# jiahuei/sparse-image-captioning

Measured on AMD Instinct MI355X. Metric: captions/sec, higher is better.
Workload: dtype bf16; 1 GPU; configs[1]: ORT dense, 256 images x 5 captions, teacher-forcing XE fwd+bwd+clip+Adam; images_per_gpu=256, regions=36, captions_per_image=5, parallelism=single

## Files before the change

### include/ortk.h

```cpp
#ifndef ORTK_H
#define ORTK_H

#include <stddef.h>
#include <stdint.h>

#ifdef __cplusplus
extern "C" {
#endif

#define ORTK_VERSION 13
#define ORTK_EINVAL (-1)
#define ORTK_ENOSPC (-2)
#define ORTK_ENOSYS (-3)
#define ORTK_EEXCHANGE (-4)

typedef void* ortk_stream;

int ortk_version(void);
int ortk_device_ok(void);

struct ortk_sparse_plan;
typedef struct ortk_config {
    int32_t d_model, d_ff, n_layers, n_heads;
    int32_t vocab, feat, seq_len;
    int32_t pad_id, bos_id, eos_id, unk_id;
    int32_t box_trig;
    int32_t precision;
    float   drop_src, drop;
    int32_t share_enc[16], share_dec[16];
    int32_t share_att_enc, share_att_dec;
    int32_t no_box;
    const struct ortk_sparse_plan* sparse_fwd;
    const struct ortk_sparse_plan* sparse_bwd;
} ortk_config;

int64_t ortk_arena_numel(const ortk_config* cfg);
int64_t ortk_arena_numel_with_buffers(const ortk_config* cfg);
int32_t ortk_arena_entries(const ortk_config* cfg);
int ortk_arena_entry(const ortk_config* cfg, int32_t index, char* name_buf, int64_t* offset,
                     int64_t* numel, int32_t* ndim, int64_t* shape, int32_t* kind);

uint32_t ortk_dropout_site_seed(uint64_t seed, int32_t stack, int32_t layer, int32_t k);

typedef struct ortk_batch {
    const float*   att_feats;
    const float*   boxes;
    const float*   att_masks;
    const int64_t* seqs;
    int64_t        seq_stride;
    const float*   tok_weight;
    int32_t B, S, R, T;
    const int32_t* cap_off;
    const int32_t* row_pos;
    int32_t        Mc;
    int32_t        no_pad_keys;
} ortk_batch;

int ortk_valid_position_tables(const int64_t* counts, int32_t R, int32_t T, int32_t* cap_off, int32_t* row_pos, ortk_stream stream);
size_t ortk_train_workspace_bytes(const ortk_config* cfg, int32_t B, int32_t S, int32_t R, int32_t T);
int ortk_valid_positions_ok(const ortk_config* cfg, int32_t B, int32_t S, int32_t R, int32_t T);

int ortk_forward(const ortk_config* cfg, const float* params, const ortk_batch* batch, void* ws, size_t ws_bytes,
                 float* logp_out, int64_t ldv, int32_t train, uint64_t seed, ortk_stream stream);
int ortk_forward_phase(const ortk_config* cfg, const float* params, const ortk_batch* batch, void* ws, size_t ws_bytes,
                       float* logp_out, int64_t ldv, int32_t train, uint64_t seed, int32_t phase, ortk_stream stream);
void* ortk_train_workspace_memory(const ortk_config* cfg, int32_t B, int32_t S, int32_t R, int32_t T, void* ws, int32_t* dtype);

int ortk_loss(const ortk_config* cfg, const ortk_batch* batch, void* ws, size_t ws_bytes,
              const float* norm_dev, float* loss_dev, ortk_stream stream);

int ortk_loss_smooth(const ortk_config* cfg, const ortk_batch* batch, void* ws, size_t ws_bytes,
                     const float* norm_dev, float* loss_dev, float smoothing, ortk_stream stream);

int ortk_loss_external(const ortk_config* cfg, const ortk_batch* batch, void* ws, size_t ws_bytes,
                       const float* logp, const float* dlogp, int64_t ldv, ortk_stream stream);

int ortk_backward(const ortk_config* cfg, const float* params, float* grads, const ortk_batch* batch,
                  void* ws, size_t ws_bytes, int32_t train, uint64_t seed, ortk_stream stream);
int ortk_backward_phase(const ortk_config* cfg, const float* params, float* grads, const ortk_batch* batch,
                        void* ws, size_t ws_bytes, int32_t train, uint64_t seed, int32_t phase, ortk_stream stream);
int64_t ortk_arena_decoder_offset(const ortk_config* cfg);

#define ORTK_SP_ELL32 0
#define ORTK_SP_ELL16 1
#define ORTK_SP_GU16  2
typedef struct ortk_sparse_block {
    int64_t src_offset;
    int64_t ld;
    int64_t stream_offset;
    int64_t capacity;
    int32_t N, K;
    int32_t chunk0;
    int32_t row0;
} ortk_sparse_block;

typedef struct ortk_sparse_plan {
    const ortk_sparse_block* blocks_host; const ortk_sparse_block* blocks_dev;
    int32_t nblocks, format;
    void* stream;
    int32_t* chunk_ptr;
    int32_t* chunk_len;
    int32_t* perm;
    int32_t* count_scratch;
    int32_t* overflow;
    int64_t total_rows;
} ortk_sparse_plan;

int ortk_sparse_build(const ortk_sparse_plan* plan, const void* dense, int32_t dtype, ortk_stream stream);

typedef struct ortk_spmm_args {
    const void* X; void* Y;
    int64_t ldx, ldy; int64_t M;
    int32_t x_dtype, y_dtype;
    const float* bias; const float* rowscale; const float* resid; int64_t ldr;
    const void* gate; int64_t ldg; int32_t gate_dtype; float gate_scale;
    int32_t relu; float drop_p; uint32_t drop_seed;
    const int32_t* drop_rows;
} ortk_spmm_args;
int ortk_spmm(const ortk_sparse_plan* plan, int32_t block, const ortk_spmm_args* a, ortk_stream stream);
int ortk_spmm_plan(const ortk_sparse_plan* plan, int32_t block, const ortk_spmm_args* a, char* buf, int32_t buf_bytes);

typedef struct ortk_chain_unit { int64_t offset, ld; } ortk_chain_unit;
typedef struct ortk_chain_args {
    const void* w16; const ortk_chain_unit* units_dev; int32_t n_units;
    void* packed; size_t packed_bytes;
    int64_t M;
    const float* x_in;
    const void* a_in; const float* bias_r; float* x_mid; uint32_t seed_r;
    const float *g1, *b1; void* y1; float* st1;
    int32_t n1; const float* bias_s1; void* out1; int64_t ld1;
    int32_t NC; const float *bias_h, *bias_o; void* h; float* x_out; uint32_t seed_h, seed_o;
    const float *g2, *b2; void* y2; float* st2;
    int32_t n2; const float* bias_s2; void* out2; int64_t ld2;
    float drop_p, eps;
    int32_t* progress;
    const int32_t* drop_rows;
} ortk_chain_args;
size_t ortk_chain_packed_bytes(int32_t n_units);
int ortk_row_chain(const ortk_chain_args* a, ortk_stream stream);

typedef struct ortk_bchain_args {
    const void* w16t; const ortk_chain_unit* units_dev; int32_t n_units;
    void* packed; size_t packed_bytes;
    int64_t M;
    int32_t nin; const void* ain; int64_t ld_ain; const void* dz0;
    const float *xa, *sta, *ga, *dresa; float *dxa, *daa, *dba; void* dza; uint32_t seed_a; int32_t mask_a;
    int32_t NC; const void* hgate; void* gh; float gate_scale;
    const float *xb, *stb, *gb, *dresb; float *dxb, *dab, *dbb; void* dzb; uint32_t seed_b; int32_t mask_b;
    int32_t n2; void* out2;
    float drop_p, eps;
    const int32_t* drop_rows;
} ortk_bchain_args;
int ortk_row_bchain(const ortk_bchain_args* a, ortk_stream stream);

typedef struct ortk_tuning {
    int32_t gemm_t64;
    int32_t attn_impl;
    int32_t attn16_min_lq;
    int32_t side_stream;
    int32_t row_chain;
    int32_t chain_wide;
    int32_t spmm_alias;
    int32_t f32_split;
    int32_t wgrad_wgs;
    int32_t wgrad_group;
    int32_t wgrad_group_splitk;
    int32_t wgrad_group_wgs;
    int32_t wgrad_group_tail;
    int32_t feats_bf16;
    int32_t ln_fuse;
    int32_t samp_epilogue;
    int32_t gemm_epilogue;
} ortk_tuning;
void ortk_get_tuning(ortk_tuning* out);
int ortk_set_tuning(const ortk_tuning* t);

#define ORTK_DEC_UNFUSED 1
#define ORTK_DEC_STACK 2
#define ORTK_DEC_SPARSE_STREAM 4
#define ORTK_DEC_STACK_RB20 8
#define ORTK_DEC_STACK_SPLIT 16
#define ORTK_DEC_SPLIT_SMALL 32
#define ORTK_DEC_SPARSE_GATHER 64
#define ORTK_DEC_STACK_FP8 128
#define ORTK_MAX_BEAM 32
typedef struct ortk_decode_opts {
    int32_t beam_size;
    int32_t num_random_sample;
    float   temperature;
    int32_t decoding_constraint;
    int32_t length_penalty;
    double  length_alpha;
    uint64_t seed;
    const struct ortk_sparse_plan* sparse;
    int32_t exec_flags;
    int32_t with_greedy;
    int64_t sample_row_offset;
    int32_t train;
    uint64_t drop_seed;
    const void* memory;
    int32_t top_k;
    float   top_p;
    int32_t group_size;
    float   diversity_lambda;
} ortk_decode_opts;

size_t ortk_decode_workspace_bytes(const ortk_config* cfg, int32_t B, int32_t S, const ortk_decode_opts* o);
int ortk_decode(const ortk_config* cfg, const float* params, const float* att_feats, const float* boxes,
                const float* att_masks, int32_t B, int32_t S, const ortk_decode_opts* o, void* ws, size_t ws_bytes,
                int64_t* seq_out, float* logprob_out, float* score_out, ortk_stream stream);
int ortk_decode_status(const void* ws, ortk_stream stream);

int ortk_encode(const ortk_config* cfg, const float* params, const float* att_feats, const float* boxes,
                const float* att_masks, int32_t B, int32_t S, void* ws, size_t ws_bytes, float* memory_out,
                ortk_stream stream);

size_t ortk_decode_step_workspace_bytes(const ortk_config* cfg, int32_t rows);
int ortk_project_memory(const ortk_config* cfg, const float* params, const float* memory, int64_t mem_rows, void* ws,
                        size_t ws_bytes, float* cross_kv, ortk_stream stream);
int ortk_decode_step(const ortk_config* cfg, const float* params, const int64_t* it, int32_t t, int32_t rows,
                     int32_t kv_groups, int32_t S, const float* cross_kv, const float* att_masks, float* self_k,
                     float* self_v, int32_t tmax, void* ws, size_t ws_bytes, float* logp_out, int64_t ld_out,
                     ortk_stream stream);


typedef struct ortk_gemm_args {
    const void* A; const void* B; void* C;
    int64_t lda, ldb, ldc;
    int32_t M, N, K, transA, transB;
    const float* bias; const float* rowscale; const float* resid; int64_t ldr;
    const void* gate; int64_t ldg; float gate_scale;
    int32_t relu; float drop_p; uint32_t drop_seed;
    int32_t accumulate, splitk, precision;
    int32_t a_dtype, b_dtype, c_dtype, gate_dtype;
    float* colsum;
    int32_t drop_row_stride, drop_row_off;
    int32_t ln_mode, ln_y_dtype;
    const float* ln_a; const float* ln_b; void* ln_y; float* ln_stats; float ln_eps;
    const float* ln_x; const float* ln_dres; float* ln_da; float* ln_db;
    float* tile_stats; int32_t stat_ncols;
    const int32_t* drop_rows;
    float* tile_samp; const int64_t* samp_seq; uint64_t samp_seed; int64_t samp_row_offset;
    int32_t samp_L, samp_t, samp_greedy_stride, samp_sample, samp_fast, samp_no_store; float samp_inv_temperature;
} ortk_gemm_args;
int ortk_gemm(const ortk_gemm_args* a, ortk_stream stream);
int ortk_gemm_plan(const ortk_gemm_args* a, char* buf, int32_t buf_bytes);
#define ORTK_WGRAD_MAX 8
typedef struct ortk_wgrad_item {
    const void* dY; int64_t lddy;
    const void* X; int64_t ldx;
    float* dW; int64_t lddw;
    float* db;
    int32_t Nout, Kin;
} ortk_wgrad_item;
typedef struct ortk_wgrad_group_args {
    ortk_wgrad_item item[ORTK_WGRAD_MAX];
    int32_t n, splitk;
    int64_t rows;
    int32_t flags;
    void* ws; size_t ws_bytes;
} ortk_wgrad_group_args;
int ortk_wgrad_group(const ortk_wgrad_group_args* a, ortk_stream stream);
size_t ortk_wgrad_group_workspace_bytes(const ortk_wgrad_group_args* a);
int ortk_prof_enable(int32_t on);
int ortk_prof_collect(int32_t key, int64_t* launches, double* total_ms, double* total_flops);
int ortk_prof_collect_bytes(int32_t key, double* total_bytes);
int ortk_prof_collect_units(int32_t key, double* total_workgroups);

int ortk_layernorm_fwd(const float* x, const float* a, const float* b, void* y, int32_t y_dtype, float* stats,
                       int64_t rows, int32_t d, float eps, ortk_stream stream);
int ortk_layernorm_bwd(const float* dy, const float* x, const float* a, const float* stats, const float* dres,
                       float* dx, float* da, float* db, int64_t rows, int32_t d, float eps, ortk_stream stream);
int ortk_layernorm_bwd_drop(const float* dy, const float* x, const float* a, const float* stats, const float* dres,
                            float* dx, float* da, float* db, int64_t rows, int32_t d, float eps, void* dz, int32_t dz_dtype,
                            float drop_p, uint32_t drop_seed, ortk_stream stream);
int ortk_layernorm_bwd_drop_rows(const float* dy, const float* x, const float* a, const float* stats, const float* dres,
                                 float* dx, float* da, float* db, int64_t rows, int32_t d, float eps, void* dz, int32_t dz_dtype,
                                 float drop_p, uint32_t drop_seed, const int32_t* drop_rows, ortk_stream stream);
int ortk_layernorm_bwd_dt(const void* dy, int32_t dy_dtype, const float* x, const float* a, const float* stats, const float* dres,
                          float* dx, float* da, float* db, int64_t rows, int32_t d, float eps, void* dz, int32_t dz_dtype,
                          float drop_p, uint32_t drop_seed, const int32_t* drop_rows, ortk_stream stream);

int ortk_box_logbias_fwd(const float* boxes, const float* const* wg, const float* const* bg, const float* dim_mat,
                         float* out, int32_t L, int32_t B, int32_t S, int32_t H, ortk_stream stream);
int ortk_box_logbias_bwd(const float* boxes, const float* const* wg, const float* const* bg, const float* dim_mat,
                         const float* dscore, float* const* dwg, float* const* dbg,
                         int32_t L, int32_t B, int32_t S, int32_t H, ortk_stream stream);
int ortk_box_embedding(const float* boxes, const float* dim_mat, float* out, int32_t B, int32_t S, ortk_stream stream);

typedef struct ortk_attn_args {
    const float* q; const float* k; const float* v; void* o;
    int64_t ldq, ldk, ldv, ldo;
    const float* kmask; const float* bias; const int32_t* kv_index;
    int64_t kv_group_stride;
    float* p;
    int32_t nkv, H, Lq, Lk, dk, causal_period;
    float drop_p; uint32_t drop_seed;
    const float* d_o; void* dq; void* d_k; void* dv; float* dscore;
    int64_t lddo, lddq, lddk, lddv;
    int32_t o_dtype, dqkv_dtype;
    int32_t kv_dtype;
    const float* k_new; const float* v_new; int64_t ld_new;
    int32_t bwd_part;
    int32_t precision;
    int32_t qkv_dtype;
    const int32_t* q_off; int32_t q_off_stride; int32_t kv_ragged;
    int32_t drop_tf_T, drop_tf_t, drop_tf_lk;
    const int32_t* drop_rows;
} ortk_attn_args;
int ortk_attention_fwd(const ortk_attn_args* a, ortk_stream stream);
int ortk_attention_bwd(const ortk_attn_args* a, ortk_stream stream);

int ortk_embed_fwd(const int64_t* seq, int64_t seq_stride, const float* lut, const float* pe, float* out, float* keymask,
                   int64_t R, int32_t T, int32_t t0, int32_t d, int32_t pad_id, float drop_p, uint32_t seed, ortk_stream stream);
int ortk_embed_bwd(const int64_t* seq, int64_t seq_stride, const float* dout, float* dlut,
                   int64_t R, int32_t T, int32_t d, float drop_p, uint32_t seed, ortk_stream stream);

int ortk_log_softmax(float* x, int64_t rows, int32_t V, int64_t ld, float scale, ortk_stream stream);
int ortk_sample_truncate(const float* logits, int64_t rows, int32_t V, int64_t ld, float temperature, int32_t top_k, float top_p,
                         const int64_t* banned, int32_t fast_exp, int32_t* kept, float* thr, int32_t* thr_col, float* kept_mass,
                         ortk_stream stream);
int ortk_beam_select(const float* logits, int64_t ld, const float* cum, const int32_t* prev, int32_t B, int32_t q, int32_t b,
                     int32_t V, int32_t fused, float scale, float* val, int32_t* parent, int32_t* token, ortk_stream stream);
int ortk_beam_select_diverse(const float* logits, int64_t ld, const float* cum, const int32_t* prev, const int32_t* pen_tok, int32_t n_pen,
                             float lambda, int32_t B, int32_t q, int32_t b, int32_t V, int32_t fused, float scale, float* val,
                             int32_t* parent, int32_t* token, float* tok_lp, ortk_stream stream);
int64_t ortk_xent_scratch_floats(int64_t rows);
int ortk_xent_fwd_bwd(const float* logits, const int64_t* targets, int64_t target_stride, int32_t T, const float* weight,
                      const float* norm_dev, float* loss_dev, float* row_loss, int64_t rows, int32_t V, int64_t ld,
                      void* dlogits, int32_t dl_dtype, int64_t ld_dl, ortk_stream stream);
int ortk_xent_smooth_fwd_bwd(const float* logits, const int64_t* targets, int64_t target_stride, int32_t T, const float* weight,
                             const float* norm_dev, float* loss_dev, float* row_loss, int64_t rows, int32_t V, int64_t ld,
                             void* dlogits, int32_t dl_dtype, int64_t ld_dl, float smoothing, ortk_stream stream);
int ortk_log_softmax_bwd(const float* logp, const float* dlogp, int64_t ld_in, void* dlogits, int32_t dl_dtype,
                         int64_t ld_out, int64_t rows, int32_t V, ortk_stream stream);

int ortk_colsum(const void* x, int32_t x_dtype, int64_t ld, float* out, int64_t M, int32_t N, ortk_stream stream);
int ortk_gate_apply(const float* x, const float* gate, void* y, int32_t y_dtype, int64_t n, float scale, ortk_stream stream);
int ortk_dropout_apply(const float* x, void* y, int32_t y_dtype, int64_t n, float p, uint32_t seed, ortk_stream stream);
int ortk_dropout_apply_rows(const float* x, void* y, int32_t y_dtype, int64_t rows, int32_t d, float p, uint32_t seed,
                            const int32_t* drop_rows, ortk_stream stream);
int ortk_cast_bf16(const float* x, void* y, int64_t n, ortk_stream stream);
int ortk_fp8_rows(const void* w16, int64_t ld, int64_t rows, int64_t n_cols, uint8_t* q, int64_t ldq, float* scale, float* deq, int64_t ldd,
                  ortk_stream stream);
int ortk_fill(float* x, int64_t n, float value, ortk_stream stream);
int ortk_axpy_cols(const void* x, void* y, int32_t dtype, int64_t ld, int64_t rows, int32_t cols, ortk_stream stream);
int64_t ortk_sum_scratch_floats(int64_t n);
int ortk_sum(const float* x, int64_t n, float* scratch, float* out_dev, ortk_stream stream);

int ortk_adam_clip(float* p, const float* g, float* m, float* v, int64_t n, float lr, float beta1, float beta2,
                   float eps, float clip, float bc1, float bc2, ortk_stream stream);
int ortk_adam_clip_zero(float* p, float* g, float* m, float* v, int64_t n, float lr, float beta1, float beta2,
                        float eps, float clip, float bc1, float bc2, ortk_stream stream);

#define ORTK_OPT_ADAM 0
#define ORTK_OPT_SGD 1
#define ORTK_OPT_SGDM 2
#define ORTK_OPT_SGDMOM 3
#define ORTK_OPT_RMSPROP 4
#define ORTK_OPT_ADAGRAD 5
typedef struct ortk_optim_args {
    float *p, *g;
    float *s1, *s2;
    int64_t n;
    int32_t kind, first_step, zero_grad;
    float lr, weight_decay, alpha, beta, eps, clip, bc1, bc2;
} ortk_optim_args;
int ortk_optim_states(int32_t kind);
int ortk_optim_step(const ortk_optim_args* a, ortk_stream stream);

int ortk_mask_apply(const float* w, const float* m, float* w_eff, int64_t n, int32_t mode, uint32_t seed, ortk_stream stream);
int ortk_mask_bwd(const float* dw_eff, const float* w, const float* m, float* dw, float* dm, int64_t n, int32_t mode,
                  uint32_t seed, const float* extra_coef_dev, ortk_stream stream);
typedef struct ortk_masked_adam_args {
    float *w, *g, *mw, *vw;
    float *ml, *mm, *mv;
    const float* draws;
    const float* active;
    const float* extra_coef;
    int64_t n, index0; int32_t mode; uint32_t seed;
    float lr_w, eps_w, lr_m, eps_m, beta1, beta2, clip, bc1, bc2;
} ortk_masked_adam_args;
int ortk_masked_adam_step(const ortk_masked_adam_args* a, ortk_stream stream);
int ortk_mask_apply_draws(const float* w, const float* m, const float* draws, float* w_eff, int64_t n, ortk_stream stream);
int ortk_mask_bwd_draws(const float* dw_eff, const float* w, const float* m, const float* draws, float* dw, float* dm, int64_t n,
                        const float* extra_coef_dev, ortk_stream stream);
int ortk_linear_block(const ortk_config* cfg, int32_t i, int64_t* offset, int32_t* N, int32_t* K);
int ortk_mask_count(const float* m, int64_t n, int32_t mode, float* count_dev, ortk_stream stream);

size_t ortk_mask_select_workspace_bytes(int32_t n_segments, int32_t n_groups, int32_t n_chunks, int32_t kind);
int ortk_mask_select(const float* w, float* mask, const int64_t* seg_offset, const int64_t* seg_numel, const int64_t* seg_group,
                     const int64_t* chunk_seg, const int64_t* chunk_start, const int64_t* chunk_len, const int64_t* n_drop,
                     int32_t n_segments, int32_t n_groups, int32_t n_chunks, int32_t kind, void* workspace, size_t workspace_bytes,
                     ortk_stream stream);

#ifdef __cplusplus
}
#endif
#endif
```

### sparse-image-captioning_amd/_lib.py

```python
import ctypes as C
import os

import torch

_HERE = os.path.dirname(os.path.abspath(__file__))
LIB_PATH = os.path.join(_HERE, "libortk.so")


class OrtkUnavailable(RuntimeError):
    pass


class OrtkError(RuntimeError):
    pass


class Config(C.Structure):
    _fields_ = [("d_model", C.c_int32), ("d_ff", C.c_int32), ("n_layers", C.c_int32), ("n_heads", C.c_int32),
                ("vocab", C.c_int32), ("feat", C.c_int32), ("seq_len", C.c_int32),
                ("pad_id", C.c_int32), ("bos_id", C.c_int32), ("eos_id", C.c_int32), ("unk_id", C.c_int32),
                ("box_trig", C.c_int32), ("precision", C.c_int32), ("drop_src", C.c_float), ("drop", C.c_float),
                ("share_enc", C.c_int32 * 16), ("share_dec", C.c_int32 * 16),
                ("share_att_enc", C.c_int32), ("share_att_dec", C.c_int32), ("no_box", C.c_int32),
                ("sparse_fwd", C.c_void_p), ("sparse_bwd", C.c_void_p)]


class Batch(C.Structure):
    _fields_ = [("att_feats", C.c_void_p), ("boxes", C.c_void_p), ("att_masks", C.c_void_p), ("seqs", C.c_void_p),
                ("seq_stride", C.c_int64), ("tok_weight", C.c_void_p),
                ("B", C.c_int32), ("S", C.c_int32), ("R", C.c_int32), ("T", C.c_int32),
                ("cap_off", C.c_void_p), ("row_pos", C.c_void_p), ("Mc", C.c_int32), ("no_pad_keys", C.c_int32)]


SP_ELL32, SP_ELL16, SP_GU16 = 0, 1, 2


class EllBlock(C.Structure):
    _fields_ = [("src_offset", C.c_int64), ("ld", C.c_int64), ("stream_offset", C.c_int64), ("capacity", C.c_int64),
                ("N", C.c_int32), ("K", C.c_int32), ("chunk0", C.c_int32), ("row0", C.c_int32)]


class EllPlanStruct(C.Structure):
    _fields_ = [("blocks_host", C.POINTER(EllBlock)), ("blocks_dev", C.c_void_p), ("nblocks", C.c_int32), ("format", C.c_int32),
                ("stream", C.c_void_p), ("chunk_ptr", C.c_void_p), ("chunk_len", C.c_void_p), ("perm", C.c_void_p),
                ("count_scratch", C.c_void_p), ("overflow", C.c_void_p), ("total_rows", C.c_int64)]


class SpmmArgs(C.Structure):
    _fields_ = [("X", C.c_void_p), ("Y", C.c_void_p), ("ldx", C.c_int64), ("ldy", C.c_int64), ("M", C.c_int64),
                ("x_dtype", C.c_int32), ("y_dtype", C.c_int32),
                ("bias", C.c_void_p), ("rowscale", C.c_void_p), ("resid", C.c_void_p), ("ldr", C.c_int64),
                ("gate", C.c_void_p), ("ldg", C.c_int64), ("gate_dtype", C.c_int32), ("gate_scale", C.c_float),
                ("relu", C.c_int32), ("drop_p", C.c_float), ("drop_seed", C.c_uint32), ("drop_rows", C.c_void_p)]


class ChainUnit(C.Structure):
    _fields_ = [("offset", C.c_int64), ("ld", C.c_int64)]


class ChainArgs(C.Structure):
    _fields_ = [("w16", C.c_void_p), ("units_dev", C.c_void_p), ("n_units", C.c_int32), ("packed", C.c_void_p), ("packed_bytes", C.c_size_t),
                ("M", C.c_int64), ("x_in", C.c_void_p),
                ("a_in", C.c_void_p), ("bias_r", C.c_void_p), ("x_mid", C.c_void_p), ("seed_r", C.c_uint32),
                ("g1", C.c_void_p), ("b1", C.c_void_p), ("y1", C.c_void_p), ("st1", C.c_void_p),
                ("n1", C.c_int32), ("bias_s1", C.c_void_p), ("out1", C.c_void_p), ("ld1", C.c_int64),
                ("NC", C.c_int32), ("bias_h", C.c_void_p), ("bias_o", C.c_void_p), ("h", C.c_void_p), ("x_out", C.c_void_p),
                ("seed_h", C.c_uint32), ("seed_o", C.c_uint32),
                ("g2", C.c_void_p), ("b2", C.c_void_p), ("y2", C.c_void_p), ("st2", C.c_void_p),
                ("n2", C.c_int32), ("bias_s2", C.c_void_p), ("out2", C.c_void_p), ("ld2", C.c_int64),
                ("drop_p", C.c_float), ("eps", C.c_float), ("progress", C.c_void_p), ("drop_rows", C.c_void_p)]


class BChainArgs(C.Structure):
    _fields_ = [("w16t", C.c_void_p), ("units_dev", C.c_void_p), ("n_units", C.c_int32), ("packed", C.c_void_p), ("packed_bytes", C.c_size_t),
                ("M", C.c_int64),
                ("nin", C.c_int32), ("ain", C.c_void_p), ("ld_ain", C.c_int64), ("dz0", C.c_void_p),
                ("xa", C.c_void_p), ("sta", C.c_void_p), ("ga", C.c_void_p), ("dresa", C.c_void_p), ("dxa", C.c_void_p), ("daa", C.c_void_p),
                ("dba", C.c_void_p), ("dza", C.c_void_p), ("seed_a", C.c_uint32), ("mask_a", C.c_int32),
                ("NC", C.c_int32), ("hgate", C.c_void_p), ("gh", C.c_void_p), ("gate_scale", C.c_float),
                ("xb", C.c_void_p), ("stb", C.c_void_p), ("gb", C.c_void_p), ("dresb", C.c_void_p), ("dxb", C.c_void_p), ("dab", C.c_void_p),
                ("dbb", C.c_void_p), ("dzb", C.c_void_p), ("seed_b", C.c_uint32), ("mask_b", C.c_int32),
                ("n2", C.c_int32), ("out2", C.c_void_p), ("drop_p", C.c_float), ("eps", C.c_float), ("drop_rows", C.c_void_p)]


class MaskedAdamArgs(C.Structure):
    _fields_ = [("w", C.c_void_p), ("g", C.c_void_p), ("mw", C.c_void_p), ("vw", C.c_void_p),
                ("ml", C.c_void_p), ("mm", C.c_void_p), ("mv", C.c_void_p),
                ("draws", C.c_void_p), ("active", C.c_void_p), ("extra_coef", C.c_void_p),
                ("n", C.c_int64), ("index0", C.c_int64), ("mode", C.c_int32), ("seed", C.c_uint32),
                ("lr_w", C.c_float), ("eps_w", C.c_float), ("lr_m", C.c_float), ("eps_m", C.c_float),
                ("beta1", C.c_float), ("beta2", C.c_float), ("clip", C.c_float), ("bc1", C.c_float), ("bc2", C.c_float)]


OPT_ADAM, OPT_SGD, OPT_SGDM, OPT_SGDMOM, OPT_RMSPROP, OPT_ADAGRAD = range(6)
OPT_KINDS = {"adam": OPT_ADAM, "sgd": OPT_SGD, "sgdm": OPT_SGDM, "sgdmom": OPT_SGDMOM, "rmsprop": OPT_RMSPROP, "adagrad": OPT_ADAGRAD}


class OptimArgs(C.Structure):
    _fields_ = [("p", C.c_void_p), ("g", C.c_void_p), ("s1", C.c_void_p), ("s2", C.c_void_p), ("n", C.c_int64),
                ("kind", C.c_int32), ("first_step", C.c_int32), ("zero_grad", C.c_int32),
                ("lr", C.c_float), ("weight_decay", C.c_float), ("alpha", C.c_float), ("beta", C.c_float), ("eps", C.c_float),
                ("clip", C.c_float), ("bc1", C.c_float), ("bc2", C.c_float)]


class Tuning(C.Structure):
    _fields_ = [("gemm_t64", C.c_int32), ("attn_impl", C.c_int32), ("attn16_min_lq", C.c_int32),
                ("side_stream", C.c_int32), ("row_chain", C.c_int32), ("chain_wide", C.c_int32), ("spmm_alias", C.c_int32), ("f32_split", C.c_int32), ("wgrad_wgs", C.c_int32),
                ("wgrad_group", C.c_int32), ("wgrad_group_splitk", C.c_int32), ("wgrad_group_wgs", C.c_int32), ("wgrad_group_tail", C.c_int32), ("feats_bf16", C.c_int32), ("ln_fuse", C.c_int32), ("samp_epilogue", C.c_int32), ("gemm_epilogue", C.c_int32)]


MAX_BEAM = 32
DEC_UNFUSED, DEC_STACK, DEC_SPARSE_STREAM, DEC_STACK_RB20, DEC_STACK_SPLIT, DEC_SPLIT_SMALL, DEC_SPARSE_GATHER, DEC_STACK_FP8 = 1, 2, 4, 8, 16, 32, 64, 128


class DecodeOpts(C.Structure):
    _fields_ = [("beam_size", C.c_int32), ("num_random_sample", C.c_int32), ("temperature", C.c_float),
                ("decoding_constraint", C.c_int32), ("length_penalty", C.c_int32), ("length_alpha", C.c_double),
                ("seed", C.c_uint64), ("sparse", C.POINTER(EllPlanStruct)), ("exec_flags", C.c_int32), ("with_greedy", C.c_int32), ("sample_row_offset", C.c_int64),
                ("train", C.c_int32), ("drop_seed", C.c_uint64), ("memory", C.c_void_p), ("top_k", C.c_int32), ("top_p", C.c_float),
                ("group_size", C.c_int32), ("diversity_lambda", C.c_float)]


class GemmArgs(C.Structure):
    _fields_ = [("A", C.c_void_p), ("B", C.c_void_p), ("C", C.c_void_p),
                ("lda", C.c_int64), ("ldb", C.c_int64), ("ldc", C.c_int64),
                ("M", C.c_int32), ("N", C.c_int32), ("K", C.c_int32), ("transA", C.c_int32), ("transB", C.c_int32),
                ("bias", C.c_void_p), ("rowscale", C.c_void_p), ("resid", C.c_void_p), ("ldr", C.c_int64),
                ("gate", C.c_void_p), ("ldg", C.c_int64), ("gate_scale", C.c_float),
                ("relu", C.c_int32), ("drop_p", C.c_float), ("drop_seed", C.c_uint32),
                ("accumulate", C.c_int32), ("splitk", C.c_int32), ("precision", C.c_int32),
                ("a_dtype", C.c_int32), ("b_dtype", C.c_int32), ("c_dtype", C.c_int32), ("gate_dtype", C.c_int32),
                ("colsum", C.c_void_p), ("drop_row_stride", C.c_int32), ("drop_row_off", C.c_int32),
                ("ln_mode", C.c_int32), ("ln_y_dtype", C.c_int32),
                ("ln_a", C.c_void_p), ("ln_b", C.c_void_p), ("ln_y", C.c_void_p), ("ln_stats", C.c_void_p), ("ln_eps", C.c_float),
                ("ln_x", C.c_void_p), ("ln_dres", C.c_void_p), ("ln_da", C.c_void_p), ("ln_db", C.c_void_p),
                ("tile_stats", C.c_void_p), ("stat_ncols", C.c_int32), ("drop_rows", C.c_void_p),
                ("tile_samp", C.c_void_p), ("samp_seq", C.c_void_p), ("samp_seed", C.c_uint64), ("samp_row_offset", C.c_int64),
                ("samp_L", C.c_int32), ("samp_t", C.c_int32), ("samp_greedy_stride", C.c_int32), ("samp_sample", C.c_int32),
                ("samp_fast", C.c_int32), ("samp_no_store", C.c_int32), ("samp_inv_temperature", C.c_float)]


class WgradItem(C.Structure):
    _fields_ = [("dY", C.c_void_p), ("lddy", C.c_int64), ("X", C.c_void_p), ("ldx", C.c_int64),
                ("dW", C.c_void_p), ("lddw", C.c_int64), ("db", C.c_void_p), ("Nout", C.c_int32), ("Kin", C.c_int32)]


WGRAD_MAX = 8


class WgradGroupArgs(C.Structure):
    _fields_ = [("item", WgradItem * WGRAD_MAX), ("n", C.c_int32), ("splitk", C.c_int32), ("rows", C.c_int64), ("flags", C.c_int32),
                ("ws", C.c_void_p), ("ws_bytes", C.c_size_t)]


class AttnArgs(C.Structure):
    _fields_ = [("q", C.c_void_p), ("k", C.c_void_p), ("v", C.c_void_p), ("o", C.c_void_p),
                ("ldq", C.c_int64), ("ldk", C.c_int64), ("ldv", C.c_int64), ("ldo", C.c_int64),
                ("kmask", C.c_void_p), ("bias", C.c_void_p), ("kv_index", C.c_void_p), ("kv_group_stride", C.c_int64),
                ("p", C.c_void_p),
                ("nkv", C.c_int32), ("H", C.c_int32), ("Lq", C.c_int32), ("Lk", C.c_int32), ("dk", C.c_int32),
                ("causal_period", C.c_int32), ("drop_p", C.c_float), ("drop_seed", C.c_uint32),
                ("d_o", C.c_void_p), ("dq", C.c_void_p), ("d_k", C.c_void_p), ("dv", C.c_void_p), ("dscore", C.c_void_p),
                ("lddo", C.c_int64), ("lddq", C.c_int64), ("lddk", C.c_int64), ("lddv", C.c_int64),
                ("o_dtype", C.c_int32), ("dqkv_dtype", C.c_int32), ("kv_dtype", C.c_int32),
                ("k_new", C.c_void_p), ("v_new", C.c_void_p), ("ld_new", C.c_int64), ("bwd_part", C.c_int32),
                ("precision", C.c_int32), ("qkv_dtype", C.c_int32),
                ("q_off", C.c_void_p), ("q_off_stride", C.c_int32), ("kv_ragged", C.c_int32),
                ("drop_tf_T", C.c_int32), ("drop_tf_t", C.c_int32), ("drop_tf_lk", C.c_int32), ("drop_rows", C.c_void_p)]


_P, _I32, _I64, _F, _U32, _U64, _SZ = C.c_void_p, C.c_int32, C.c_int64, C.c_float, C.c_uint32, C.c_uint64, C.c_size_t
_CFG = C.POINTER(Config)

SIGNATURES = {
    "ortk_version": (_I32, []),
    "ortk_device_ok": (_I32, []),
    "ortk_arena_numel": (_I64, [_CFG]),
    "ortk_arena_numel_with_buffers": (_I64, [_CFG]),
    "ortk_arena_entries": (_I32, [_CFG]),
    "ortk_arena_entry": (_I32, [_CFG, _I32, C.c_char_p, C.POINTER(_I64), C.POINTER(_I64), C.POINTER(_I32),
                               C.POINTER(_I64), C.POINTER(_I32)]),
    "ortk_train_workspace_bytes": (_SZ, [_CFG, _I32, _I32, _I32, _I32]),
    "ortk_valid_positions_ok": (_I32, [_CFG, _I32, _I32, _I32, _I32]),
    "ortk_forward": (_I32, [_CFG, _P, C.POINTER(Batch), _P, _SZ, _P, _I64, _I32, _U64, _P]),
    "ortk_forward_phase": (_I32, [_CFG, _P, C.POINTER(Batch), _P, _SZ, _P, _I64, _I32, _U64, _I32, _P]),
    "ortk_train_workspace_memory": (_P, [_CFG, _I32, _I32, _I32, _I32, _P, C.POINTER(C.c_int32)]),
    "ortk_loss": (_I32, [_CFG, C.POINTER(Batch), _P, _SZ, _P, _P, _P]),
    "ortk_loss_smooth": (_I32, [_CFG, C.POINTER(Batch), _P, _SZ, _P, _P, _F, _P]),
    "ortk_loss_external": (_I32, [_CFG, C.POINTER(Batch), _P, _SZ, _P, _P, _I64, _P]),
    "ortk_backward": (_I32, [_CFG, _P, _P, C.POINTER(Batch), _P, _SZ, _I32, _U64, _P]),
    "ortk_backward_phase": (_I32, [_CFG, _P, _P, C.POINTER(Batch), _P, _SZ, _I32, _U64, _I32, _P]),
    "ortk_arena_decoder_offset": (_I64, [_CFG]),
    "ortk_decode_workspace_bytes": (_SZ, [_CFG, _I32, _I32, C.POINTER(DecodeOpts)]),
    "ortk_decode": (_I32, [_CFG, _P, _P, _P, _P, _I32, _I32, C.POINTER(DecodeOpts), _P, _SZ, _P, _P, _P, _P]),
    "ortk_decode_status": (_I32, [_P, _P]),
    "ortk_encode": (_I32, [_CFG, _P, _P, _P, _P, _I32, _I32, _P, _SZ, _P, _P]),
    "ortk_chain_packed_bytes": (_SZ, [_I32]),
    "ortk_row_chain": (_I32, [C.POINTER(ChainArgs), _P]),
    "ortk_row_bchain": (_I32, [C.POINTER(BChainArgs), _P]),
    "ortk_get_tuning": (None, [C.POINTER(Tuning)]),
    "ortk_set_tuning": (_I32, [C.POINTER(Tuning)]),
    "ortk_gemm": (_I32, [C.POINTER(GemmArgs), _P]),
    "ortk_gemm_plan": (_I32, [C.POINTER(GemmArgs), C.c_char_p, _I32]),
    "ortk_wgrad_group": (_I32, [C.POINTER(WgradGroupArgs), _P]),
    "ortk_wgrad_group_workspace_bytes": (_SZ, [C.POINTER(WgradGroupArgs)]),
    "ortk_prof_enable": (_I32, [_I32]),
    "ortk_prof_collect": (_I32, [_I32, C.POINTER(_I64), C.POINTER(C.c_double), C.POINTER(C.c_double)]),
    "ortk_prof_collect_bytes": (_I32, [_I32, C.POINTER(C.c_double)]),
    "ortk_prof_collect_units": (_I32, [_I32, C.POINTER(C.c_double)]),
    "ortk_layernorm_fwd": (_I32, [_P, _P, _P, _P, _I32, _P, _I64, _I32, _F, _P]),
    "ortk_layernorm_bwd": (_I32, [_P, _P, _P, _P, _P, _P, _P, _P, _I64, _I32, _F, _P]),
    "ortk_layernorm_bwd_drop": (_I32, [_P, _P, _P, _P, _P, _P, _P, _P, _I64, _I32, _F, _P, _I32, _F, C.c_uint32, _P]),
    "ortk_layernorm_bwd_drop_rows": (_I32, [_P, _P, _P, _P, _P, _P, _P, _P, _I64, _I32, _F, _P, _I32, _F, C.c_uint32, _P, _P]),
    "ortk_layernorm_bwd_dt": (_I32, [_P, _I32, _P, _P, _P, _P, _P, _P, _P, _I64, _I32, _F, _P, _I32, _F, C.c_uint32, _P, _P]),
    "ortk_box_logbias_fwd": (_I32, [_P, C.POINTER(_P), C.POINTER(_P), C.POINTER(_F), _P, _I32, _I32, _I32, _I32, _P]),
    "ortk_box_logbias_bwd": (_I32, [_P, C.POINTER(_P), C.POINTER(_P), C.POINTER(_F), _P, C.POINTER(_P), C.POINTER(_P),
                                   _I32, _I32, _I32, _I32, _P]),
    "ortk_box_embedding": (_I32, [_P, C.POINTER(_F), _P, _I32, _I32, _P]),
    "ortk_attention_fwd": (_I32, [C.POINTER(AttnArgs), _P]),
    "ortk_attention_bwd": (_I32, [C.POINTER(AttnArgs), _P]),
    "ortk_valid_position_tables": (_I32, [_P, _I32, _I32, _P, _P, _P]),
    "ortk_embed_fwd": (_I32, [_P, _I64, _P, _P, _P, _P, _I64, _I32, _I32, _I32, _I32, _F, _U32, _P]),
    "ortk_embed_bwd": (_I32, [_P, _I64, _P, _P, _I64, _I32, _I32, _F, _U32, _P]),
    "ortk_log_softmax": (_I32, [_P, _I64, _I32, _I64, _F, _P]),
    "ortk_sample_truncate": (_I32, [_P, _I64, _I32, _I64, _F, _I32, _F, _P, _I32, _P, _P, _P, _P, _P]),
    "ortk_beam_select": (_I32, [_P, _I64, _P, _P, _I32, _I32, _I32, _I32, _I32, _F, _P, _P, _P, _P]),
    "ortk_beam_select_diverse": (_I32, [_P, _I64, _P, _P, _P, _I32, _F, _I32, _I32, _I32, _I32, _I32, _F, _P, _P, _P, _P, _P]),
    "ortk_xent_scratch_floats": (_I64, [_I64]),
    "ortk_xent_fwd_bwd": (_I32, [_P, _P, _I64, _I32, _P, _P, _P, _P, _I64, _I32, _I64, _P, _I32, _I64, _P]),
    "ortk_xent_smooth_fwd_bwd": (_I32, [_P, _P, _I64, _I32, _P, _P, _P, _P, _I64, _I32, _I64, _P, _I32, _I64, _F, _P]),
    "ortk_log_softmax_bwd": (_I32, [_P, _P, _I64, _P, _I32, _I64, _I64, _I32, _P]),
    "ortk_colsum": (_I32, [_P, _I32, _I64, _P, _I64, _I32, _P]),
    "ortk_gate_apply": (_I32, [_P, _P, _P, _I32, _I64, _F, _P]),
    "ortk_dropout_apply": (_I32, [_P, _P, _I32, _I64, _F, _U32, _P]),
    "ortk_dropout_apply_rows": (_I32, [_P, _P, _I32, _I64, _I32, _F, _U32, _P, _P]),
    "ortk_dropout_site_seed": (_U32, [_U64, _I32, _I32, _I32]),
    "ortk_cast_bf16": (_I32, [_P, _P, _I64, _P]),
    "ortk_fp8_rows": (_I32, [_P, _I64, _I64, _I64, _P, _I64, _P, _P, _I64, _P]),
    "ortk_fill": (_I32, [_P, _I64, _F, _P]),
    "ortk_sum_scratch_floats": (_I64, [_I64]),
    "ortk_sum": (_I32, [_P, _I64, _P, _P, _P]),
    "ortk_adam_clip": (_I32, [_P, _P, _P, _P, _I64, _F, _F, _F, _F, _F, _F, _F, _P]),
    "ortk_adam_clip_zero": (_I32, [_P, _P, _P, _P, _I64, _F, _F, _F, _F, _F, _F, _F, _P]),
    "ortk_optim_states": (_I32, [_I32]),
    "ortk_optim_step": (_I32, [C.POINTER(OptimArgs), _P]),
    "ortk_mask_apply": (_I32, [_P, _P, _P, _I64, _I32, _U32, _P]),
    "ortk_mask_bwd": (_I32, [_P, _P, _P, _P, _P, _I64, _I32, _U32, _P, _P]),
    "ortk_masked_adam_step": (_I32, [C.POINTER(MaskedAdamArgs), _P]),
    "ortk_mask_count": (_I32, [_P, _I64, _I32, _P, _P]),
    "ortk_mask_select_workspace_bytes": (_SZ, [_I32, _I32, _I32, _I32]),
    "ortk_mask_select": (_I32, [_P, _P, _P, _P, _P, _P, _P, _P, _P, _I32, _I32, _I32, _I32, _P, _SZ, _P]),
    "ortk_mask_apply_draws": (_I32, [_P, _P, _P, _P, _I64, _P]),
    "ortk_mask_bwd_draws": (_I32, [_P, _P, _P, _P, _P, _P, _I64, _P, _P]),
    "ortk_decode_step_workspace_bytes": (_SZ, [_CFG, _I32]),
    "ortk_project_memory": (_I32, [_CFG, _P, _P, _I64, _P, _SZ, _P, _P]),
    "ortk_decode_step": (_I32, [_CFG, _P, _P, _I32, _I32, _I32, _I32, _P, _P, _P, _P, _I32, _P, _SZ, _P, _I64, _P]),
    "ortk_axpy_cols": (_I32, [_P, _P, _I32, _I64, _I64, _I32, _P]),
    "ortk_linear_block": (_I32, [_CFG, _I32, C.POINTER(C.c_int64), C.POINTER(C.c_int32), C.POINTER(C.c_int32)]),
    "ortk_sparse_build": (_I32, [C.POINTER(EllPlanStruct), _P, _I32, _P]),
    "ortk_spmm": (_I32, [C.POINTER(EllPlanStruct), _I32, C.POINTER(SpmmArgs), _P]),
    "ortk_spmm_plan": (_I32, [C.POINTER(EllPlanStruct), _I32, C.POINTER(SpmmArgs), C.c_char_p, _I32]),
}

_lib = None
ABI_VERSION = 13


def lib():
    global _lib
    if _lib is None:
        if not os.path.exists(LIB_PATH):
            raise OrtkUnavailable(
                f"{LIB_PATH} is missing: build it with `python -c 'import __graft_entry__ as g; g.build()'` "
                "(or `make -C sparse-image-captioning_amd/csrc`).  There is no CPU / PyTorch fallback.")
        h = C.CDLL(LIB_PATH)
        h.ortk_version.restype = C.c_int32
        if h.ortk_version() != ABI_VERSION:
            raise OrtkUnavailable(
                f"{LIB_PATH} is ABI version {h.ortk_version()}, these bindings were written for version {ABI_VERSION} (include/ortk.h: "
                "ORTK_VERSION): a stale build.  Rebuild it with `make -C sparse-image-captioning_amd/csrc`.")
        for name, (res, args) in SIGNATURES.items():
            fn = getattr(h, name)
            fn.restype = res
            fn.argtypes = args
        _lib = h
    return _lib


def set_tuning(**kw):
    t = Tuning()
    lib().ortk_get_tuning(C.byref(t))
    old = {f: getattr(t, f) for f, _ in Tuning._fields_}
    for k, v in kw.items():
        assert k in old, k
        setattr(t, k, int(v))
    check(lib().ortk_set_tuning(C.byref(t)), "ortk_set_tuning")
    return old


def gemm_plan(args):
    buf = C.create_string_buffer(256)
    check(lib().ortk_gemm_plan(C.byref(args), buf, len(buf)), "ortk_gemm_plan")
    return [k for k in buf.value.decode().split(";") if k]


def spmm_plan(plan, block, args):
    if hasattr(plan, "ref"):
        plan = plan.ref()
    elif isinstance(plan, EllPlanStruct):
        plan = C.pointer(plan)
    buf = C.create_string_buffer(128)
    check(lib().ortk_spmm_plan(plan, block, C.byref(args), buf, len(buf)), "ortk_spmm_plan")
    return buf.value.decode()


def require_gpu():
    if not torch.cuda.is_available():
        raise OrtkUnavailable("no HIP device visible: the ORT hot path runs only on MI355X (gfx950); no CPU fallback")
    if not lib().ortk_device_ok():
        raise OrtkUnavailable("the visible device is not gfx950; libortk.so carries gfx950 code objects only")


def stream_ptr():
    return C.c_void_p(torch.cuda.current_stream().cuda_stream)


def ptr(t):
    if t is None:
        return None
    assert t.is_cuda, "libortk takes device pointers only"
    return C.c_void_p(t.data_ptr())


def check(code, what):
    if code != 0:
        names = {-1: "ORTK_EINVAL (bad argument / unsupported shape)", -2: "ORTK_ENOSPC (workspace too small)",
                 -3: "ORTK_ENOSYS (option not implemented)",
                 -4: "ORTK_EEXCHANGE (column-split decode: an exchange group never met — the launch was not fully resident; "
                     "outputs are poisoned; set model.exclusive_gpu = False when the GPU is shared)"}
        raise OrtkError(f"{what} failed: {names.get(code, 'hipError ' + str(code))}")


def f32c(t):
    assert t.is_cuda
    if t.dtype != torch.float32:
        t = t.float()
    return t.contiguous()
```

### sparse-image-captioning_amd/csrc/ortk_attn16.hip

```cpp
#include <cstdlib>
#include "ortk_internal.h"

namespace {

constexpr int P16 = 72;

__device__ __forceinline__ void wsync() { __builtin_amdgcn_fence(__ATOMIC_ACQ_REL, "wavefront"); __builtin_amdgcn_wave_barrier(); }

template <int NJT> struct KeyGeo {
    static constexpr int KJ = NJT <= 2 ? 32 : NJT <= 4 ? 64 : NJT <= 6 ? 96 : 128;
    static constexpr int PJ = NJT <= 4 ? P16 : 136;
};

template <int PITCH = P16>
__device__ __forceinline__ bf16x8 frag_row(const __bf16* img, int row, int k0) {
    return *reinterpret_cast<const bf16x8*>(img + row * PITCH + k0);
}
template <int PITCH = P16>
__device__ __forceinline__ bf16x8 frag_tr(const __bf16* img, int k0, int x0, int lane) {
    const int lr = lane & 15, lq = lane >> 4;
    const __bf16* p = img + (k0 + 8 * lq + (lr >> 2)) * PITCH + x0 + 4 * (lane & 3);
    typedef bf16x4 __attribute__((address_space(3))) * lds4;
    const bf16x4 lo = __builtin_amdgcn_ds_read_tr16_b64_v4bf16((lds4)(p));
    const bf16x4 hi = __builtin_amdgcn_ds_read_tr16_b64_v4bf16((lds4)(p + 4 * PITCH));
    return (bf16x8){lo[0], lo[1], lo[2], lo[3], hi[0], hi[1], hi[2], hi[3]};
}
__device__ __forceinline__ bf16x4 cvt4(float4 v) { return (bf16x4){(__bf16)v.x, (__bf16)v.y, (__bf16)v.z, (__bf16)v.w}; }
__device__ __forceinline__ bf16x8 cvt8(float4 a, float4 b) {
    return (bf16x8){(__bf16)a.x, (__bf16)a.y, (__bf16)a.z, (__bf16)a.w, (__bf16)b.x, (__bf16)b.y, (__bf16)b.z, (__bf16)b.w};
}
__device__ __forceinline__ f32x4 mma(bf16x8 x, bf16x8 y, f32x4 acc) { return __builtin_amdgcn_mfma_f32_16x16x32_bf16(x, y, acc, 0, 0, 0); }

template <int DKT>
__device__ __forceinline__ void stage_rows(__bf16* img, const float* src, int64_t ld, int rows, int rows_pad, int tid, int nthr) {
    constexpr int CPR = DKT / 4;
    for (int idx = tid; idx < rows_pad * CPR; idx += nthr) {
        const int r = idx / CPR, c = (idx % CPR) * 4;
        float4 v = make_float4(0.f, 0.f, 0.f, 0.f);
        if (r < rows) v = *reinterpret_cast<const float4*>(src + (int64_t)r * ld + c);
        *reinterpret_cast<bf16x4*>(img + r * (DKT + 8) + c) = cvt4(v);
    }
}
template <int DKT>
__device__ __forceinline__ void stage_rows(__bf16* img, const __bf16* src, int64_t ld, int rows, int rows_pad, int tid, int nthr) {
    constexpr int CPR = DKT / 8;
    for (int idx = tid; idx < rows_pad * CPR; idx += nthr) {
        const int r = idx / CPR, c = (idx % CPR) * 8;
        bf16x8 v = (bf16x8){0, 0, 0, 0, 0, 0, 0, 0};
        if (r < rows) v = *reinterpret_cast<const bf16x8*>(src + (int64_t)r * ld + c);
        *reinterpret_cast<bf16x8*>(img + r * (DKT + 8) + c) = v;
    }
}
__device__ __forceinline__ bf16x8 ld_frag(const float* p) { return cvt8(*reinterpret_cast<const float4*>(p), *reinterpret_cast<const float4*>(p + 4)); }
__device__ __forceinline__ bf16x8 ld_frag(const __bf16* p) { return *reinterpret_cast<const bf16x8*>(p); }

template <int NJT, typename TQ, int DKT>
__global__ __launch_bounds__(512) void attn16_fwd_kernel(ortk_attn_args a) {
    constexpr int DK = DKT, PD = DKT + 8;
    const float qscale = DKT == 64 ? 0.125f : 0.17677669529663687f;
    const TQ* aq = reinterpret_cast<const TQ*>(a.q); const TQ* ak = reinterpret_cast<const TQ*>(a.k); const TQ* av = reinterpret_cast<const TQ*>(a.v);
    extern __shared__ __attribute__((aligned(16))) __bf16 sm16[];
    const int tid = threadIdx.x, lane = tid & 63, wave = tid >> 6, nw = blockDim.x >> 6;
    const int g = blockIdx.x / a.H, h = blockIdx.x - g * a.H;
    const int Lk = a.Lk, Lq = a.Lq;
    constexpr int KJ = KeyGeo<NJT>::KJ, PJ = KeyGeo<NJT>::PJ;
    __bf16* sK = sm16;
    __bf16* sV = sK + 16 * NJT * PD;
    __bf16* sP = sV + KJ * PD + wave * 16 * PJ;
    float* sMask = reinterpret_cast<float*>(sm16 + (16 * NJT + KJ) * PD + 16 * nw * PJ);
    const int lr = lane & 15, lq = lane >> 4;
    const bool vec_p = (Lk & 3) == 0;
    const int nit = (Lq + 15) >> 4;
    const int64_t qrow0 = a.q_off ? (int64_t)a.q_off[(int64_t)g * a.q_off_stride] : (int64_t)g * Lq;
    const int Lqg = a.q_off ? min(Lq, (int)(a.q_off[(int64_t)(g + 1) * a.q_off_stride] - qrow0)) : Lq;
    const int64_t krow0 = (a.q_off && a.kv_ragged) ? qrow0 : (int64_t)g * Lk;
    const int Lkg = (a.q_off && a.kv_ragged) ? min(Lk, Lqg) : Lk;
    const int it = wave;
    const int i = it * 16 + lr;
    const bool iv = it < nit && i < Lqg;
    const int64_t prow = (((int64_t)g * a.H + h) * Lq + i) * Lk;
    const int64_t drow = (a.drop_rows && a.q_off && iv && a.drop_p > 0.f)
                             ? (((int64_t)g * a.H + h) * Lq + ((int64_t)a.drop_rows[qrow0 + i] - (int64_t)g * Lq)) * Lk : prow;
    bf16x8 qf[DK / 32];
#pragma unroll
    for (int ks = 0; ks < DK / 32; ++ks) qf[ks] = (bf16x8){0, 0, 0, 0, 0, 0, 0, 0};
    if (iv) {
        const TQ* qp = aq + (qrow0 + i) * a.ldq + h * DK + 8 * lq;
#pragma unroll
        for (int ks = 0; ks < DK / 32; ++ks) qf[ks] = ld_frag(qp + 32 * ks);
    }
    float4 bias4[NJT];
#pragma unroll
    for (int jt = 0; jt < NJT; ++jt) {
        const int j0 = 16 * jt + 4 * lq;
        bias4[jt] = make_float4(0.f, 0.f, 0.f, 0.f);
        if (a.bias && iv) {
            if (vec_p && j0 < Lk) bias4[jt] = *reinterpret_cast<const float4*>(a.bias + prow + j0);
            else { float* bp = &bias4[jt].x; for (int r = 0; r < 4; ++r) if (j0 + r < Lk) bp[r] = a.bias[prow + j0 + r]; }
        }
    }
    stage_rows<DK>(sK, ak + krow0 * a.ldk + h * DK, a.ldk, Lkg, 16 * NJT, tid, blockDim.x);
    stage_rows<DK>(sV, av + krow0 * a.ldv + h * DK, a.ldv, Lkg, KJ, tid, blockDim.x);
    for (int j = tid; j < 128; j += blockDim.x)
        sMask[j] = (j < Lkg) ? (a.kmask ? a.kmask[krow0 + j] : 1.f) : -1.f;
    for (int idx = lane; idx < 16 * (KJ / 4); idx += 64)
        *reinterpret_cast<bf16x4*>(sP + (idx / (KJ / 4)) * PJ + (idx % (KJ / 4)) * 4) = cvt4(make_float4(0.f, 0.f, 0.f, 0.f));
    __syncthreads();
    const float inv_keep = a.drop_p > 0.f ? 1.f / (1.f - a.drop_p) : 1.f;
    if (it < nit) {
        f32x4 s[NJT];
#pragma unroll
        for (int jt = 0; jt < NJT; ++jt) {
            s[jt] = (f32x4){0.f, 0.f, 0.f, 0.f};
#pragma unroll
            for (int ks = 0; ks < DK / 32; ++ks) s[jt] = mma(frag_row<PD>(sK, 16 * jt + lr, 32 * ks + 8 * lq), qf[ks], s[jt]);
        }
        const int qpos = a.causal_period > 0 ? i % a.causal_period : 0;
        float mx = -INFINITY;
#pragma unroll
        for (int jt = 0; jt < NJT; ++jt) {
            const int j0 = 16 * jt + 4 * lq;
            const float bb[4] = {bias4[jt].x, bias4[jt].y, bias4[jt].z, bias4[jt].w};
#pragma unroll
            for (int r = 0; r < 4; ++r) {
                const int j = j0 + r;
                const float mk = sMask[j];
                float x = s[jt][r] * qscale;
                if (mk == 0.f || (a.causal_period > 0 && j > qpos)) x = -1e9f;
                if (mk < 0.f) x = -INFINITY;
                else if (a.bias && iv) x = bb[r] + x;
                s[jt][r] = x;
                mx = fmaxf(mx, x);
            }
        }
        mx = fmaxf(mx, __shfl_xor(mx, 16, 64)); mx = fmaxf(mx, __shfl_xor(mx, 32, 64));
        float sum = 0.f;
#pragma unroll
        for (int jt = 0; jt < NJT; ++jt)
#pragma unroll
            for (int r = 0; r < 4; ++r) { const float e = expf(s[jt][r] - mx); s[jt][r] = e; sum += e; }
        sum += __shfl_xor(sum, 16, 64); sum += __shfl_xor(sum, 32, 64);
#pragma unroll
        for (int jt = 0; jt < NJT; ++jt) {
            const int j0 = 16 * jt + 4 * lq;
            float p[4];
#pragma unroll
            for (int r = 0; r < 4; ++r) p[r] = (iv && j0 + r < Lk) ? s[jt][r] / sum : 0.f;
            if (a.p && iv) {
                if (vec_p && j0 < Lk) *reinterpret_cast<float4*>(a.p + prow + j0) = make_float4(p[0], p[1], p[2], p[3]);
                else for (int r = 0; r < 4; ++r) if (j0 + r < Lk) a.p[prow + j0 + r] = p[r];
            }
            if (a.drop_p > 0.f) {
                bool kp[4];
                ortk_keep4(a.drop_seed, (uint64_t)(drow + j0), a.drop_p, kp);
#pragma unroll
                for (int r = 0; r < 4; ++r) p[r] = kp[r] ? p[r] * inv_keep : 0.f;
            }
            *reinterpret_cast<bf16x4*>(sP + lr * PJ + j0) = cvt4(make_float4(p[0], p[1], p[2], p[3]));
        }
        wsync();
        bf16x8 pf[KJ / 32];
#pragma unroll
        for (int ks = 0; ks < KJ / 32; ++ks) pf[ks] = frag_row<PJ>(sP, lr, 32 * ks + 8 * lq);
#pragma unroll
        for (int dt = 0; dt < DK / 16; ++dt) {
            f32x4 o = (f32x4){0.f, 0.f, 0.f, 0.f};
#pragma unroll
            for (int ks = 0; ks < KJ / 32; ++ks) o = mma(frag_tr<PD>(sV, 32 * ks, 16 * dt, lane), pf[ks], o);
            if (iv) st_elem4(a.o, (qrow0 + i) * a.ldo + h * DK + 16 * dt + 4 * lq, a.o_dtype, make_float4(o[0], o[1], o[2], o[3]));
        }
    }
}
static int key_kj(int njt) { return njt <= 2 ? 32 : njt <= 4 ? 64 : njt <= 6 ? 96 : 128; }
static int key_pj(int njt) { return njt <= 4 ? P16 : 136; }
static size_t fwd16_lds(int njt, int nw, int dk) {
    return ((size_t)(16 * njt + key_kj(njt)) * (dk + 8) + (size_t)16 * nw * key_pj(njt)) * sizeof(__bf16) + 128 * sizeof(float);
}

template <int NJT, typename TQ, int DKT>
__global__ __launch_bounds__(512) void attn16_bwd_kernel(ortk_attn_args a, int Lqp) {
    constexpr int DK = DKT, PD = DKT + 8;
    const float qscale = DKT == 64 ? 0.125f : 0.17677669529663687f;
    const TQ* aq = reinterpret_cast<const TQ*>(a.q); const TQ* ak = reinterpret_cast<const TQ*>(a.k); const TQ* av = reinterpret_cast<const TQ*>(a.v);
    extern __shared__ __attribute__((aligned(16))) __bf16 sm16[];
    const int tid = threadIdx.x, lane = tid & 63, wave = tid >> 6, nw = blockDim.x >> 6;
    const int g = blockIdx.x / a.H, h = blockIdx.x - g * a.H;
    const int Lk = a.Lk, Lq = a.Lq;
    constexpr int KJ = KeyGeo<NJT>::KJ, PJ = KeyGeo<NJT>::PJ;
    __bf16* sK = sm16;
    __bf16* sV = sK + KJ * PD;
    __bf16* sQ = sV + 16 * NJT * PD;
    __bf16* sG = sQ + Lqp * PD;
    __bf16* sS = sG + Lqp * PD;
    __bf16* sD = sS + Lqp * PJ;
    const int lr = lane & 15, lq = lane >> 4;
    const bool vec_p = (Lk & 3) == 0;
    const int nit = (Lq + 15) >> 4;
    const int64_t qrow0 = a.q_off ? (int64_t)a.q_off[(int64_t)g * a.q_off_stride] : (int64_t)g * Lq;
    const int Lqg = a.q_off ? min(Lq, (int)(a.q_off[(int64_t)(g + 1) * a.q_off_stride] - qrow0)) : Lq;
    const int64_t krow0 = (a.q_off && a.kv_ragged) ? qrow0 : (int64_t)g * Lk;
    const int Lkg = (a.q_off && a.kv_ragged) ? min(Lk, Lqg) : Lk;
    const int it = wave;
    const int i0 = it * 16, i = i0 + lr;
    const bool iv = it < nit && i < Lqg;
    const int64_t prow = (((int64_t)g * a.H + h) * Lq + i) * Lk;
    const int64_t drow = (a.drop_rows && a.q_off && iv && a.drop_p > 0.f)
                             ? (((int64_t)g * a.H + h) * Lq + ((int64_t)a.drop_rows[qrow0 + i] - (int64_t)g * Lq)) * Lk : prow;
    float4 praw[NJT];
#pragma unroll
    for (int jt = 0; jt < NJT; ++jt) {
        const int j0 = 16 * jt + 4 * lq;
        praw[jt] = make_float4(0.f, 0.f, 0.f, 0.f);
        if (iv) {
            if (vec_p && j0 < Lk) praw[jt] = *reinterpret_cast<const float4*>(a.p + prow + j0);
            else { float* q = &praw[jt].x; for (int r = 0; r < 4; ++r) if (j0 + r < Lk) q[r] = a.p[prow + j0 + r]; }
        }
    }
    stage_rows<DK>(sK, ak + krow0 * a.ldk + h * DK, a.ldk, Lkg, KJ, tid, blockDim.x);
    stage_rows<DK>(sV, av + krow0 * a.ldv + h * DK, a.ldv, Lkg, 16 * NJT, tid, blockDim.x);
    stage_rows<DK>(sQ, aq + qrow0 * a.ldq + h * DK, a.ldq, Lqg, Lqp, tid, blockDim.x);
    stage_rows<DK>(sG, reinterpret_cast<const TQ*>(a.d_o) + qrow0 * a.lddo + h * DK, a.lddo, Lqg, Lqp, tid, blockDim.x);
    for (int idx = tid; idx < 2 * Lqp * (KJ / 4); idx += blockDim.x)
        *reinterpret_cast<bf16x4*>(sS + (idx / (KJ / 4)) * PJ + (idx % (KJ / 4)) * 4) = cvt4(make_float4(0.f, 0.f, 0.f, 0.f));
    __syncthreads();
    const float inv_keep = a.drop_p > 0.f ? 1.f / (1.f - a.drop_p) : 1.f;
    if (it < nit) {
        bf16x8 gf[DK / 32];
#pragma unroll
        for (int ks = 0; ks < DK / 32; ++ks) gf[ks] = frag_row<PD>(sG, i, 32 * ks + 8 * lq);
        f32x4 dp[NJT], pp[NJT];
        float dot = 0.f;
#pragma unroll
        for (int jt = 0; jt < NJT; ++jt) {
            dp[jt] = (f32x4){0.f, 0.f, 0.f, 0.f};
#pragma unroll
            for (int ks = 0; ks < DK / 32; ++ks) dp[jt] = mma(frag_row<PD>(sV, 16 * jt + lr, 32 * ks + 8 * lq), gf[ks], dp[jt]);
            const int j0 = 16 * jt + 4 * lq;
            const float pv[4] = {praw[jt].x, praw[jt].y, praw[jt].z, praw[jt].w};
            float pd[4];
            bool kp[4] = {true, true, true, true};
            if (a.drop_p > 0.f) ortk_keep4(a.drop_seed, (uint64_t)(drow + j0), a.drop_p, kp);
#pragma unroll
            for (int r = 0; r < 4; ++r) {
                const bool valid = iv && j0 + r < Lk;
                const bool keep = valid && kp[r];
                const float d = keep ? dp[jt][r] * inv_keep : 0.f;
                pd[r] = keep ? pv[r] * inv_keep : 0.f;
                pp[jt][r] = valid ? pv[r] : 0.f; dp[jt][r] = d; dot += pp[jt][r] * d;
            }
            *reinterpret_cast<bf16x4*>(sD + i * PJ + j0) = cvt4(make_float4(pd[0], pd[1], pd[2], pd[3]));
        }
        dot += __shfl_xor(dot, 16, 64); dot += __shfl_xor(dot, 32, 64);
#pragma unroll
        for (int jt = 0; jt < NJT; ++jt) {
            const int j0 = 16 * jt + 4 * lq;
            float ds[4];
#pragma unroll
            for (int r = 0; r < 4; ++r) ds[r] = pp[jt][r] * (dp[jt][r] - dot);
            if (a.dscore && iv) {
                if (vec_p && j0 < Lk) *reinterpret_cast<float4*>(a.dscore + prow + j0) = make_float4(ds[0], ds[1], ds[2], ds[3]);
                else for (int r = 0; r < 4; ++r) if (j0 + r < Lk) a.dscore[prow + j0 + r] = ds[r];
            }
            *reinterpret_cast<bf16x4*>(sS + i * PJ + j0) = cvt4(make_float4(ds[0] * qscale, ds[1] * qscale, ds[2] * qscale, ds[3] * qscale));
        }
        wsync();
        bf16x8 sf[KJ / 32];
#pragma unroll
        for (int ks = 0; ks < KJ / 32; ++ks) sf[ks] = frag_row<PJ>(sS, i, 32 * ks + 8 * lq);
#pragma unroll
        for (int dt = 0; dt < DK / 16; ++dt) {
            f32x4 acc = (f32x4){0.f, 0.f, 0.f, 0.f};
#pragma unroll
            for (int ks = 0; ks < KJ / 32; ++ks) acc = mma(frag_tr<PD>(sK, 32 * ks, 16 * dt, lane), sf[ks], acc);
            if (iv) st_elem4(a.dq, (qrow0 + i) * a.lddq + h * DK + 16 * dt + 4 * lq, a.dqkv_dtype, make_float4(acc[0], acc[1], acc[2], acc[3]));
        }
    }
    __syncthreads();
    constexpr int NDT = DK / 16;
    const int ntiles = 2 * NJT * NDT;
    for (int t = wave; t < ntiles; t += nw) {
        const int which = t / (NJT * NDT), rem = t - which * NJT * NDT, jt = rem / NDT, dt = rem % NDT;
        const __bf16* sA = which == 0 ? sS : sD;
        const __bf16* sB = which == 0 ? sQ : sG;
        f32x4 acc = (f32x4){0.f, 0.f, 0.f, 0.f};
        for (int k0 = 0; k0 < Lqp; k0 += 32) acc = mma(frag_tr<PD>(sB, k0, 16 * dt, lane), frag_tr<PJ>(sA, k0, 16 * jt, lane), acc);
        const int j = 16 * jt + lr;
        if (j < Lkg) {
            const int64_t row = krow0 + j;
            const float4 v = make_float4(acc[0], acc[1], acc[2], acc[3]);
            if (which == 0) st_elem4(a.d_k, row * a.lddk + h * DK + 16 * dt + 4 * lq, a.dqkv_dtype, v);
            else            st_elem4(a.dv, row * a.lddv + h * DK + 16 * dt + 4 * lq, a.dqkv_dtype, v);
        }
    }
}
static size_t bwd16_lds(int njt, int Lqp, int dk) {
    return ((size_t)(key_kj(njt) + 16 * njt + 2 * Lqp) * (dk + 8) + (size_t)2 * Lqp * key_pj(njt)) * sizeof(__bf16);
}

bool al16(const void* p) { return (reinterpret_cast<uintptr_t>(p) & 15) == 0; }

}

namespace ortk {

bool attn16_shape_ok(int Lq, int Lk, int dk) { return (dk == 64 || dk == 32) && Lk >= 1 && Lk <= 128 && Lq >= 1 && Lq <= 128; }

bool attn16_ok(const ortk_attn_args* a, bool bwd) {
    const int min_lq = ortk::tuning().attn16_min_lq;
    if (a->precision != 1 || !attn16_shape_ok(a->Lq, a->Lk, a->dk) || (a->qkv_dtype == 0 && a->Lq < min_lq && a->Lk <= 48)) return false;
    if (a->kv_index || a->kv_group_stride > 0 || a->kv_dtype != 0 || a->k_new || a->v_new) return false;
    if (a->q_off && (a->qkv_dtype != 1 || a->q_off_stride < 1)) return false;
    if ((a->ldq | a->ldk | a->ldv) % (a->qkv_dtype ? 8 : 4) || !al16(a->q) || !al16(a->k) || !al16(a->v)) return false;
    if (!bwd) {
        const int64_t eo = a->o_dtype == ORTK_BF16 ? 2 : 4;
        if (a->ldo % 4 || (reinterpret_cast<uintptr_t>(a->o) % (4 * eo)) || (a->p && !al16(a->p)) || (a->bias && !al16(a->bias))) return false;
    } else {
        const int64_t eg = a->dqkv_dtype == ORTK_BF16 ? 2 : 4;
        if (!a->p || !a->d_o || !a->dq || !a->d_k || !a->dv) return false;
        if ((a->lddo % (a->qkv_dtype ? 8 : 4)) || (a->lddq | a->lddk | a->lddv) % 4 || !al16(a->d_o) || !al16(a->p) || (a->dscore && !al16(a->dscore))) return false;
        if ((reinterpret_cast<uintptr_t>(a->dq) | reinterpret_cast<uintptr_t>(a->d_k) | reinterpret_cast<uintptr_t>(a->dv)) % (4 * eg)) return false;
    }
    return true;
}

typedef void (*fwd16_fn)(ortk_attn_args);
typedef void (*bwd16_fn)(ortk_attn_args, int);
template <typename TQ, int DKT> static fwd16_fn pick_fwd(int njt) {
    switch (njt) {
        case 1: return attn16_fwd_kernel<1, TQ, DKT>; case 2: return attn16_fwd_kernel<2, TQ, DKT>; case 3: return attn16_fwd_kernel<3, TQ, DKT>;
        case 4: return attn16_fwd_kernel<4, TQ, DKT>; case 5: return attn16_fwd_kernel<5, TQ, DKT>; case 6: return attn16_fwd_kernel<6, TQ, DKT>;
        case 7: return attn16_fwd_kernel<7, TQ, DKT>; default: return attn16_fwd_kernel<8, TQ, DKT>;
    }
}
template <typename TQ, int DKT> static bwd16_fn pick_bwd(int njt) {
    switch (njt) {
        case 1: return attn16_bwd_kernel<1, TQ, DKT>; case 2: return attn16_bwd_kernel<2, TQ, DKT>; case 3: return attn16_bwd_kernel<3, TQ, DKT>;
        case 4: return attn16_bwd_kernel<4, TQ, DKT>; case 5: return attn16_bwd_kernel<5, TQ, DKT>; case 6: return attn16_bwd_kernel<6, TQ, DKT>;
        case 7: return attn16_bwd_kernel<7, TQ, DKT>; default: return attn16_bwd_kernel<8, TQ, DKT>;
    }
}

int attn16_fwd(const ortk_attn_args* a, hipStream_t s) {
    const int njt = (a->Lk + 15) / 16, nw = (a->Lq + 15) / 16;
    const fwd16_fn fn = a->dk == 64 ? (a->qkv_dtype ? pick_fwd<__bf16, 64>(njt) : pick_fwd<float, 64>(njt))
                                    : (a->qkv_dtype ? pick_fwd<__bf16, 32>(njt) : pick_fwd<float, 32>(njt));
    const size_t lds = fwd16_lds(njt, nw, a->dk);
    if (lds > 64 * 1024) ortk::lds_attr(reinterpret_cast<const void*>(fn), 160 * 1024);
    hipLaunchKernelGGL(fn, dim3((unsigned)(a->nkv * a->H)), dim3(64 * nw), lds, s, *a);
    ORTK_CHECK_LAUNCH();
    return 0;
}

int attn16_bwd(const ortk_attn_args* a, hipStream_t s) {
    const int njt = (a->Lk + 15) / 16, nw = (a->Lq + 15) / 16, Lqp = (int)ortk_align(a->Lq, 32);
    const bwd16_fn fn = a->dk == 64 ? (a->qkv_dtype ? pick_bwd<__bf16, 64>(njt) : pick_bwd<float, 64>(njt))
                                    : (a->qkv_dtype ? pick_bwd<__bf16, 32>(njt) : pick_bwd<float, 32>(njt));
    const size_t lds = bwd16_lds(njt, Lqp, a->dk);
    if (lds > 160 * 1024) return ORTK_EINVAL;
    if (lds > 64 * 1024) ortk::lds_attr(reinterpret_cast<const void*>(fn), 160 * 1024);
    hipLaunchKernelGGL(fn, dim3((unsigned)(a->nkv * a->H)), dim3(64 * nw), lds, s, *a, Lqp);
    ORTK_CHECK_LAUNCH();
    return 0;
}

}
```

### sparse-image-captioning_amd/csrc/ortk_runtime.hip

```cpp
#include <mutex>
#include <vector>
#include "ortk_internal.h"

namespace ortk {
static ortk_tuning tuning_defaults() {
    ortk_tuning t{};
    t.gemm_t64 = 640;
    t.attn_impl = 0;
    t.attn16_min_lq = 33;
    t.side_stream = 1;
    t.row_chain = 1;
    t.chain_wide = 1;
    t.spmm_alias = 1;
    t.f32_split = 1;
    t.wgrad_wgs = 384;
    t.wgrad_group = 3;
    t.wgrad_group_splitk = 0;
    t.wgrad_group_wgs = 80;
    t.wgrad_group_tail = 1;
    t.feats_bf16 = 1;
    t.ln_fuse = 0;
    t.samp_epilogue = 1;
    t.gemm_epilogue = 0;
    return t;
}
static ortk_tuning g_tuning = tuning_defaults();
const ortk_tuning& tuning() { return g_tuning; }
}

extern "C" void ortk_get_tuning(ortk_tuning* out) { if (out) *out = ortk::g_tuning; }
extern "C" int ortk_set_tuning(const ortk_tuning* t) {
    if (!t) return ORTK_EINVAL;
    auto in = [](int32_t v, int32_t lo, int32_t hi) { return v >= lo && v <= hi; };
    if (!in(t->attn_impl, 0, 4) || t->attn16_min_lq < 1 || !in(t->f32_split, 0, 7) || t->wgrad_wgs < 1 ||
        !in(t->wgrad_group, 0, 15) || !in(t->wgrad_group_splitk, 0, 8) || t->wgrad_group_wgs < 1 || !in(t->wgrad_group_tail, 0, 1) ||
        !in(t->feats_bf16, 0, 1) || !in(t->ln_fuse, 0, 15) || (t->ln_fuse & 2)  ||
        !in(t->samp_epilogue, 0, 1) || !in(t->gemm_epilogue, 0, 3)) return ORTK_EINVAL;
    ortk::g_tuning = *t;
    return 0;
}

namespace ortk {
int lds_attr(const void* fn, size_t bytes) {
    struct Key { int dev; const void* fn; size_t bytes; };
    static std::mutex mu;
    static std::vector<Key>* seen = new std::vector<Key>();
    int dev = 0;
    if (hipGetDevice(&dev) != hipSuccess) return ORTK_EINVAL;
    std::lock_guard<std::mutex> lk(mu);
    for (const Key& k : *seen) if (k.dev == dev && k.fn == fn && k.bytes >= bytes) return 0;
    if (hipFuncSetAttribute(fn, hipFuncAttributeMaxDynamicSharedMemorySize, (int)bytes) != hipSuccess) return ORTK_EINVAL;
    seen->push_back(Key{dev, fn, bytes});
    return 0;
}
}

namespace {
struct ProfRec { hipEvent_t a, b; int key; double flops, bytes; int slot; double per_count; double units; };
constexpr int PROF_SLOTS = 1 << 16;
unsigned long long* g_prof_slots = nullptr;
int g_prof_slot_next = 0;
bool g_prof_on = false;
bool g_prof_serial = false;
std::mutex g_prof_mu;
std::vector<ProfRec>* g_prof = nullptr;
}

namespace ortk {
bool ortk_prof_active() { return g_prof_on; }
bool ortk_prof_serial() { return g_prof_serial; }
bool prof_begin(int key, double flops, double bytes, hipStream_t s, ProfMark& m) {
    m.live = false;
    if (!g_prof_on) return false;
    if (hipEventCreate(&m.a) != hipSuccess) return false;
    if (hipEventCreate(&m.b) != hipSuccess) { (void)hipEventDestroy(m.a); return false; }
    m.key = key; m.flops = flops; m.bytes = bytes; m.live = true;
    (void)hipEventRecord(m.a, s);
    return true;
}
void prof_end(const ProfMark& m, hipStream_t s) {
    if (!m.live) return;
    (void)hipEventRecord(m.b, s);
    ProfRec rec{m.a, m.b, m.key, m.flops, m.bytes, m.slot, m.per_count, m.units};
    std::lock_guard<std::mutex> lk(g_prof_mu);
    g_prof->push_back(rec);
}
unsigned long long* prof_slot(int* index) {
    if (index) *index = -1;
    if (!g_prof_on || !g_prof_slots || !index) return nullptr;
    std::lock_guard<std::mutex> lk(g_prof_mu);
    if (g_prof_slot_next >= PROF_SLOTS) return nullptr;
    *index = g_prof_slot_next++;
    return g_prof_slots + *index;
}
}

extern "C" int ortk_prof_enable(int32_t on) {
    if (!g_prof) g_prof = new std::vector<ProfRec>();
    for (auto& r : *g_prof) { (void)hipEventDestroy(r.a); (void)hipEventDestroy(r.b); }
    g_prof->clear();
    if (on && !g_prof_slots && hipMalloc(reinterpret_cast<void**>(&g_prof_slots), PROF_SLOTS * sizeof(unsigned long long)) != hipSuccess) g_prof_slots = nullptr;
    if (on && g_prof_slots && hipMemset(g_prof_slots, 0, PROF_SLOTS * sizeof(unsigned long long)) != hipSuccess) return ORTK_EINVAL;
    g_prof_slot_next = 0;
    g_prof_on = on != 0;
    g_prof_serial = on == 1;
    return 0;
}
extern "C" int ortk_prof_collect(int32_t key, int64_t* launches, double* total_ms, double* total_flops) {
    if (!g_prof || !launches || !total_ms || !total_flops) return ORTK_EINVAL;
    *launches = 0; *total_ms = 0; *total_flops = 0;
    for (auto& r : *g_prof) {
        if (r.key != key) continue;
        if (hipEventSynchronize(r.b) != hipSuccess) return ORTK_EINVAL;
        float ms = 0.f;
        if (hipEventElapsedTime(&ms, r.a, r.b) != hipSuccess) return ORTK_EINVAL;
        *launches += 1; *total_ms += ms; *total_flops += r.flops;
    }
    return 0;
}

extern "C" int ortk_prof_collect_units(int32_t key, double* total_workgroups) {
    if (!g_prof || !total_workgroups) return ORTK_EINVAL;
    *total_workgroups = 0;
    for (auto& r : *g_prof) if (r.key == key) *total_workgroups += r.units;
    return 0;
}

extern "C" int ortk_prof_collect_bytes(int32_t key, double* total_bytes) {
    if (!g_prof || !total_bytes) return ORTK_EINVAL;
    *total_bytes = 0;
    std::vector<unsigned long long> slots;
    if (g_prof_slots && g_prof_slot_next > 0) {
        slots.resize((size_t)g_prof_slot_next);
        if (hipMemcpy(slots.data(), g_prof_slots, slots.size() * sizeof(unsigned long long), hipMemcpyDeviceToHost) != hipSuccess) return ORTK_EINVAL;
    }
    for (auto& r : *g_prof) {
        if (r.key != key) continue;
        *total_bytes += r.bytes;
        if (r.slot >= 0 && (size_t)r.slot < slots.size()) *total_bytes += r.per_count * (double)slots[(size_t)r.slot];
    }
    return 0;
}
```

Baseline: 127,900 captions/sec.

## Add short-sequence attn16 kernels mapping one wave per caption-head pair

Adds specialised forward and backward attention kernels for sequences of at most 32 tokens with bf16 inputs. Each wave handles one (caption, head) pair and keeps K/V fragments in registers instead of staging them through block-wide LDS with __syncthreads. The aim is to cut block-level synchronisation and idle waves for the short caption sequences (length 17) used in teacher-forcing. A new tuning knob enables it by default with 4 waves per block; the ABI version is bumped.

```diff
diff --git a/include/ortk.h b/include/ortk.h
--- a/include/ortk.h
+++ b/include/ortk.h
@@ -8,7 +8,7 @@
 extern "C" {
 #endif
 
-#define ORTK_VERSION 13
+#define ORTK_VERSION 14
 #define ORTK_EINVAL (-1)
 #define ORTK_ENOSPC (-2)
 #define ORTK_ENOSYS (-3)
@@ -171,6 +171,7 @@
     int32_t ln_fuse;
     int32_t samp_epilogue;
     int32_t gemm_epilogue;
+    int32_t attn16_short;
 } ortk_tuning;
 void ortk_get_tuning(ortk_tuning* out);
 int ortk_set_tuning(const ortk_tuning* t);
diff --git a/scratch/attn16_short_bench.py b/scratch/attn16_short_bench.py
--- /dev/null
+++ b/scratch/attn16_short_bench.py
@@ -0,0 +1,56 @@
+import ctypes as C, hashlib, os, socket, sys
+import torch
+ROOT = os.path.dirname(os.path.dirname(os.path.abspath(__file__)))
+sys.path.insert(0, ROOT)
+import sparse_image_captioning_amd as P
+L = P._lib
+L.require_gpu()
+print("box", socket.gethostname(), " lib md5", hashlib.md5(open(L.LIB_PATH, "rb").read()).hexdigest(), flush=True)
+ncap, H, T, dk = 1280, 8, 17, 64
+d = H * dk
+
+
+def case(name, lengths):
+    off = [0]
+    for n in lengths: off.append(off[-1] + n)
+    M = off[-1]
+    g = torch.Generator().manual_seed(3)
+    qkv = torch.randn(M, 3 * d, generator=g).bfloat16().cuda()
+    do = torch.randn(M, d, generator=g).bfloat16().cuda()
+    o = torch.empty(M, d, device="cuda", dtype=torch.bfloat16); dqkv = torch.empty(M, 3 * d, device="cuda", dtype=torch.bfloat16)
+    p = torch.zeros(ncap, H, T, T, device="cuda"); km = torch.ones(M, device="cuda")
+    a = L.AttnArgs()
+    a.precision, a.qkv_dtype, a.o_dtype, a.dqkv_dtype = 1, 1, 1, 1
+    a.q, a.k, a.v = qkv.data_ptr(), qkv.data_ptr() + 2 * d, qkv.data_ptr() + 4 * d
+    a.o, a.p, a.kmask = o.data_ptr(), p.data_ptr(), km.data_ptr()
+    a.ldq = a.ldk = a.ldv = 3 * d; a.ldo = d
+    a.nkv, a.H, a.Lq, a.Lk, a.dk, a.causal_period, a.drop_p, a.drop_seed = ncap, H, T, T, dk, T, 0.1, 5
+    a.d_o, a.dq, a.d_k, a.dv = do.data_ptr(), dqkv.data_ptr(), dqkv.data_ptr() + 2 * d, dqkv.data_ptr() + 4 * d
+    a.lddo = d; a.lddq = a.lddk = a.lddv = 3 * d
+    if lengths != [T] * ncap:
+        qo = torch.tensor(off, dtype=torch.int32).cuda()
+        a.q_off, a.q_off_stride, a.kv_ragged = qo.data_ptr(), 1, 1
+    fns = (("fwd", L.lib().ortk_attention_fwd), ("bwd", L.lib().ortk_attention_bwd))
+    res, sums = {}, {}
+    for rep in range(3):
+        for sw in (0, 4, 8):
+            L.set_tuning(attn16_short=sw)
+            for fname, fn in fns:
+                for _ in range(3): L.check(fn(C.byref(a), L.stream_ptr()), fname)
+                torch.cuda.synchronize()
+                e0, e1 = torch.cuda.Event(enable_timing=True), torch.cuda.Event(enable_timing=True)
+                e0.record()
+                for _ in range(50): fn(C.byref(a), L.stream_ptr())
+                e1.record(); torch.cuda.synchronize()
+                res.setdefault((sw, fname), []).append(e0.elapsed_time(e1) * 20)
+            sums[sw] = [hashlib.md5(t.cpu().view(torch.int16).numpy().tobytes()).hexdigest() for t in (o, dqkv)] + \
+                       [hashlib.md5(p.cpu().numpy().tobytes()).hexdigest()]
+    L.set_tuning(attn16_short=1)
+    for sw in (0, 4, 8):
+        print(f"{name:8s} attn16_short={sw}: fwd us {' '.join(f'{x:6.1f}' for x in res[(sw, 'fwd')])}   bwd us {' '.join(f'{x:6.1f}' for x in res[(sw, 'bwd')])}"
+              f"   outputs {'== attn16_short=0' if sums[sw] == sums[0] else 'DIFFER'}", flush=True)
+
+
+case("padded", [T] * ncap)
+gl = torch.Generator().manual_seed(11)
+case("valid", torch.randint(9, T + 1, (ncap,), generator=gl).tolist())
diff --git a/sparse-image-captioning_amd/_lib.py b/sparse-image-captioning_amd/_lib.py
--- a/sparse-image-captioning_amd/_lib.py
+++ b/sparse-image-captioning_amd/_lib.py
@@ -106,7 +106,7 @@
 class Tuning(C.Structure):
     _fields_ = [("gemm_t64", C.c_int32), ("attn_impl", C.c_int32), ("attn16_min_lq", C.c_int32),
                 ("side_stream", C.c_int32), ("row_chain", C.c_int32), ("chain_wide", C.c_int32), ("spmm_alias", C.c_int32), ("f32_split", C.c_int32), ("wgrad_wgs", C.c_int32),
-                ("wgrad_group", C.c_int32), ("wgrad_group_splitk", C.c_int32), ("wgrad_group_wgs", C.c_int32), ("wgrad_group_tail", C.c_int32), ("feats_bf16", C.c_int32), ("ln_fuse", C.c_int32), ("samp_epilogue", C.c_int32), ("gemm_epilogue", C.c_int32)]
+                ("wgrad_group", C.c_int32), ("wgrad_group_splitk", C.c_int32), ("wgrad_group_wgs", C.c_int32), ("wgrad_group_tail", C.c_int32), ("feats_bf16", C.c_int32), ("ln_fuse", C.c_int32), ("samp_epilogue", C.c_int32), ("gemm_epilogue", C.c_int32), ("attn16_short", C.c_int32)]
 
 
 MAX_BEAM = 32
@@ -263,7 +263,7 @@
 }
 
 _lib = None
-ABI_VERSION = 13
+ABI_VERSION = 14
 
 
 def lib():
diff --git a/sparse-image-captioning_amd/csrc/ortk_attn16.hip b/sparse-image-captioning_amd/csrc/ortk_attn16.hip
--- a/sparse-image-captioning_amd/csrc/ortk_attn16.hip
+++ b/sparse-image-captioning_amd/csrc/ortk_attn16.hip
@@ -54,10 +54,132 @@
 __device__ __forceinline__ bf16x8 ld_frag(const float* p) { return cvt8(*reinterpret_cast<const float4*>(p), *reinterpret_cast<const float4*>(p + 4)); }
 __device__ __forceinline__ bf16x8 ld_frag(const __bf16* p) { return *reinterpret_cast<const bf16x8*>(p); }
 
+template <int PD> struct LdsRowFrags {
+    const __bf16* img; int lr, lq;
+    __device__ __forceinline__ bf16x8 operator()(int jt, int ks) const { return frag_row<PD>(img, 16 * jt + lr, 32 * ks + 8 * lq); }
+};
+template <int NJT, int NKS> struct RegRowFrags {
+    bf16x8 f[NJT][NKS];
+    __device__ __forceinline__ bf16x8 operator()(int jt, int ks) const { return f[jt][ks]; }
+};
+template <int NJT, int NKS>
+__device__ __forceinline__ void ld_row_frags(RegRowFrags<NJT, NKS>& out, const __bf16* src, int64_t ld, int rows, int lane) {
+    const int lr = lane & 15, lq = lane >> 4;
+#pragma unroll
+    for (int jt = 0; jt < NJT; ++jt)
+#pragma unroll
+        for (int ks = 0; ks < NKS; ++ks) {
+            out.f[jt][ks] = (bf16x8){0, 0, 0, 0, 0, 0, 0, 0};
+            if (16 * jt + lr < rows) out.f[jt][ks] = ld_frag(src + (int64_t)(16 * jt + lr) * ld + 32 * ks + 8 * lq);
+        }
+}
+template <int NJT>
+__device__ __forceinline__ void ld_keys4(float4 (&out)[NJT], const float* base, bool on, int64_t prow, int Lk, int lq) {
+    const bool vec_p = (Lk & 3) == 0;
+#pragma unroll
+    for (int jt = 0; jt < NJT; ++jt) {
+        const int j0 = 16 * jt + 4 * lq;
+        out[jt] = make_float4(0.f, 0.f, 0.f, 0.f);
+        if (on) {
+            if (vec_p && j0 < Lk) out[jt] = *reinterpret_cast<const float4*>(base + prow + j0);
+            else { float* q = &out[jt].x; for (int r = 0; r < 4; ++r) if (j0 + r < Lk) q[r] = base[prow + j0 + r]; }
+        }
+    }
+}
+template <int DKT>
+__device__ __forceinline__ void stage32_ld(bf16x8 (&v)[DKT / 16], const __bf16* src, int64_t ld, int rows, int lane) {
+    constexpr int CPR = DKT / 8;
+#pragma unroll
+    for (int n = 0; n < DKT / 16; ++n) {
+        const int idx = lane + 64 * n, r = idx / CPR, c = (idx % CPR) * 8;
+        v[n] = (bf16x8){0, 0, 0, 0, 0, 0, 0, 0};
+        if (r < rows) v[n] = *reinterpret_cast<const bf16x8*>(src + (int64_t)r * ld + c);
+    }
+}
+template <int DKT>
+__device__ __forceinline__ void stage32_st(__bf16* img, const bf16x8 (&v)[DKT / 16], int lane) {
+    constexpr int CPR = DKT / 8;
+#pragma unroll
+    for (int n = 0; n < DKT / 16; ++n) {
+        const int idx = lane + 64 * n, r = idx / CPR, c = (idx % CPR) * 8;
+        *reinterpret_cast<bf16x8*>(img + r * (DKT + 8) + c) = v[n];
+    }
+}
+
+template <int NJT, int DKT, int PJ, typename KF>
+__device__ __forceinline__ void fwd16_tile(const ortk_attn_args& a, const KF& kfr, const bf16x8 (&qf)[DKT / 32], const float4 (&bias4)[NJT],
+                                           const float* sMask, const __bf16* sV, __bf16* sP, int lane, int i, bool iv,
+                                           int64_t prow, int64_t drow, int64_t orow, int h, float inv_keep) {
+    constexpr int DK = DKT, PD = DKT + 8, KJ = KeyGeo<NJT>::KJ;
+    const float qscale = DKT == 64 ? 0.125f : 0.17677669529663687f;
+    const int lr = lane & 15, lq = lane >> 4, Lk = a.Lk;
+    const bool vec_p = (Lk & 3) == 0;
+    f32x4 s[NJT];
+#pragma unroll
+    for (int jt = 0; jt < NJT; ++jt) {
+        s[jt] = (f32x4){0.f, 0.f, 0.f, 0.f};
+#pragma unroll
+        for (int ks = 0; ks < DK / 32; ++ks) s[jt] = mma(kfr(jt, ks), qf[ks], s[jt]);
+    }
+    const int qpos = a.causal_period > 0 ? i % a.causal_period : 0;
+    float mx = -INFINITY;
+#pragma unroll
+    for (int jt = 0; jt < NJT; ++jt) {
+        const int j0 = 16 * jt + 4 * lq;
+        const float bb[4] = {bias4[jt].x, bias4[jt].y, bias4[jt].z, bias4[jt].w};
+#pragma unroll
+        for (int r = 0; r < 4; ++r) {
+            const int j = j0 + r;
+            const float mk = sMask[j];
+            float x = s[jt][r] * qscale;
+            if (mk == 0.f || (a.causal_period > 0 && j > qpos)) x = -1e9f;
+            if (mk < 0.f) x = -INFINITY;
+            else if (a.bias && iv) x = bb[r] + x;
+            s[jt][r] = x;
+            mx = fmaxf(mx, x);
+        }
+    }
+    mx = fmaxf(mx, __shfl_xor(mx, 16, 64)); mx = fmaxf(mx, __shfl_xor(mx, 32, 64));
+    float sum = 0.f;
+#pragma unroll
+    for (int jt = 0; jt < NJT; ++jt)
+#pragma unroll
+        for (int r = 0; r < 4; ++r) { const float e = expf(s[jt][r] - mx); s[jt][r] = e; sum += e; }
+    sum += __shfl_xor(sum, 16, 64); sum += __shfl_xor(sum, 32, 64);
+#pragma unroll
+    for (int jt = 0; jt < NJT; ++jt) {
+        const int j0 = 16 * jt + 4 * lq;
+        float p[4];
+#pragma unroll
+        for (int r = 0; r < 4; ++r) p[r] = (iv && j0 + r < Lk) ? s[jt][r] / sum : 0.f;
+        if (a.p && iv) {
+            if (vec_p && j0 < Lk) *reinterpret_cast<float4*>(a.p + prow + j0) = make_float4(p[0], p[1], p[2], p[3]);
+            else for (int r = 0; r < 4; ++r) if (j0 + r < Lk) a.p[prow + j0 + r] = p[r];
+        }
+        if (a.drop_p > 0.f) {
+            bool kp[4];
+            ortk_keep4(a.drop_seed, (uint64_t)(drow + j0), a.drop_p, kp);
+#pragma unroll
+            for (int r = 0; r < 4; ++r) p[r] = kp[r] ? p[r] * inv_keep : 0.f;
+        }
+        *reinterpret_cast<bf16x4*>(sP + lr * PJ + j0) = cvt4(make_float4(p[0], p[1], p[2], p[3]));
+    }
+    wsync();
+    bf16x8 pf[KJ / 32];
+#pragma unroll
+    for (int ks = 0; ks < KJ / 32; ++ks) pf[ks] = frag_row<PJ>(sP, lr, 32 * ks + 8 * lq);
+#pragma unroll
+    for (int dt = 0; dt < DK / 16; ++dt) {
+        f32x4 o = (f32x4){0.f, 0.f, 0.f, 0.f};
+#pragma unroll
+        for (int ks = 0; ks < KJ / 32; ++ks) o = mma(frag_tr<PD>(sV, 32 * ks, 16 * dt, lane), pf[ks], o);
+        if (iv) st_elem4(a.o, orow * a.ldo + h * DK + 16 * dt + 4 * lq, a.o_dtype, make_float4(o[0], o[1], o[2], o[3]));
+    }
+}
+
 template <int NJT, typename TQ, int DKT>
 __global__ __launch_bounds__(512) void attn16_fwd_kernel(ortk_attn_args a) {
     constexpr int DK = DKT, PD = DKT + 8;
-    const float qscale = DKT == 64 ? 0.125f : 0.17677669529663687f;
     const TQ* aq = reinterpret_cast<const TQ*>(a.q); const TQ* ak = reinterpret_cast<const TQ*>(a.k); const TQ* av = reinterpret_cast<const TQ*>(a.v);
     extern __shared__ __attribute__((aligned(16))) __bf16 sm16[];
     const int tid = threadIdx.x, lane = tid & 63, wave = tid >> 6, nw = blockDim.x >> 6;
@@ -69,7 +191,6 @@
     __bf16* sP = sV + KJ * PD + wave * 16 * PJ;
     float* sMask = reinterpret_cast<float*>(sm16 + (16 * NJT + KJ) * PD + 16 * nw * PJ);
     const int lr = lane & 15, lq = lane >> 4;
-    const bool vec_p = (Lk & 3) == 0;
     const int nit = (Lq + 15) >> 4;
     const int64_t qrow0 = a.q_off ? (int64_t)a.q_off[(int64_t)g * a.q_off_stride] : (int64_t)g * Lq;
     const int Lqg = a.q_off ? min(Lq, (int)(a.q_off[(int64_t)(g + 1) * a.q_off_stride] - qrow0)) : Lq;
@@ -90,15 +211,7 @@
         for (int ks = 0; ks < DK / 32; ++ks) qf[ks] = ld_frag(qp + 32 * ks);
     }
     float4 bias4[NJT];
-#pragma unroll
-    for (int jt = 0; jt < NJT; ++jt) {
-        const int j0 = 16 * jt + 4 * lq;
-        bias4[jt] = make_float4(0.f, 0.f, 0.f, 0.f);
-        if (a.bias && iv) {
-            if (vec_p && j0 < Lk) bias4[jt] = *reinterpret_cast<const float4*>(a.bias + prow + j0);
-            else { float* bp = &bias4[jt].x; for (int r = 0; r < 4; ++r) if (j0 + r < Lk) bp[r] = a.bias[prow + j0 + r]; }
-        }
-    }
+    ld_keys4<NJT>(bias4, a.bias, a.bias && iv, prow, Lk, lq);
     stage_rows<DK>(sK, ak + krow0 * a.ldk + h * DK, a.ldk, Lkg, 16 * NJT, tid, blockDim.x);
     stage_rows<DK>(sV, av + krow0 * a.ldv + h * DK, a.ldv, Lkg, KJ, tid, blockDim.x);
     for (int j = tid; j < 128; j += blockDim.x)
@@ -107,68 +220,73 @@
         *reinterpret_cast<bf16x4*>(sP + (idx / (KJ / 4)) * PJ + (idx % (KJ / 4)) * 4) = cvt4(make_float4(0.f, 0.f, 0.f, 0.f));
     __syncthreads();
     const float inv_keep = a.drop_p > 0.f ? 1.f / (1.f - a.drop_p) : 1.f;
-    if (it < nit) {
-        f32x4 s[NJT];
-#pragma unroll
-        for (int jt = 0; jt < NJT; ++jt) {
-            s[jt] = (f32x4){0.f, 0.f, 0.f, 0.f};
-#pragma unroll
-            for (int ks = 0; ks < DK / 32; ++ks) s[jt] = mma(frag_row<PD>(sK, 16 * jt + lr, 32 * ks + 8 * lq), qf[ks], s[jt]);
-        }
-        const int qpos = a.causal_period > 0 ? i % a.causal_period : 0;
-        float mx = -INFINITY;
-#pragma unroll
-        for (int jt = 0; jt < NJT; ++jt) {
-            const int j0 = 16 * jt + 4 * lq;
-            const float bb[4] = {bias4[jt].x, bias4[jt].y, bias4[jt].z, bias4[jt].w};
-#pragma unroll
-            for (int r = 0; r < 4; ++r) {
-                const int j = j0 + r;
-                const float mk = sMask[j];
-                float x = s[jt][r] * qscale;
-                if (mk == 0.f || (a.causal_period > 0 && j > qpos)) x = -1e9f;
-                if (mk < 0.f) x = -INFINITY;
-                else if (a.bias && iv) x = bb[r] + x;
-                s[jt][r] = x;
-                mx = fmaxf(mx, x);
-            }
-        }
-        mx = fmaxf(mx, __shfl_xor(mx, 16, 64)); mx = fmaxf(mx, __shfl_xor(mx, 32, 64));
-        float sum = 0.f;
-#pragma unroll
-        for (int jt = 0; jt < NJT; ++jt)
-#pragma unroll
-            for (int r = 0; r < 4; ++r) { const float e = expf(s[jt][r] - mx); s[jt][r] = e; sum += e; }
-        sum += __shfl_xor(sum, 16, 64); sum += __shfl_xor(sum, 32, 64);
-#pragma unroll
-        for (int jt = 0; jt < NJT; ++jt) {
-            const int j0 = 16 * jt + 4 * lq;
-            float p[4];
-#pragma unroll
-            for (int r = 0; r < 4; ++r) p[r] = (iv && j0 + r < Lk) ? s[jt][r] / sum : 0.f;
-            if (a.p && iv) {
-                if (vec_p && j0 < Lk) *reinterpret_cast<float4*>(a.p + prow + j0) = make_float4(p[0], p[1], p[2], p[3]);
-                else for (int r = 0; r < 4; ++r) if (j0 + r < Lk) a.p[prow + j0 + r] = p[r];
-            }
-            if (a.drop_p > 0.f) {
-                bool kp[4];
-                ortk_keep4(a.drop_seed, (uint64_t)(drow + j0), a.drop_p, kp);
-#pragma unroll
-                for (int r = 0; r < 4; ++r) p[r] = kp[r] ? p[r] * inv_keep : 0.f;
-            }
-            *reinterpret_cast<bf16x4*>(sP + lr * PJ + j0) = cvt4(make_float4(p[0], p[1], p[2], p[3]));
-        }
+    if (it < nit)
+        fwd16_tile<NJT, DKT, PJ>(a, LdsRowFrags<PD>{sK, lr, lq}, qf, bias4, sMask, sV, sP, lane, i, iv, prow, drow, qrow0 + i, h, inv_keep);
+}
+
+constexpr int KJS = 32, PJS = KJS + 8;
+template <int DKT> constexpr int fwd16s_wave_elems() { return KJS * (DKT + 8) + 16 * PJS + 64; }
+template <int NJT, int DKT>
+__global__ __launch_bounds__(512) void attn16s_fwd_kernel(ortk_attn_args a) {
+    static_assert(NJT <= 2, "the short kernels serve at most 32 keys");
+    constexpr int DK = DKT, PD = DKT + 8, NKS = DKT / 32;
+    const __bf16* aq = reinterpret_cast<const __bf16*>(a.q); const __bf16* ak = reinterpret_cast<const __bf16*>(a.k); const __bf16* av = reinterpret_cast<const __bf16*>(a.v);
+    extern __shared__ __attribute__((aligned(16))) __bf16 sm16[];
+    const int lane = threadIdx.x & 63, wave = __builtin_amdgcn_readfirstlane((int)(threadIdx.x >> 6)), W = blockDim.x >> 6;
+    const int pair = blockIdx.x * W + wave;
+    if (pair >= a.nkv * a.H) return;
+    const int g = pair / a.H, h = pair - g * a.H;
+    const int Lk = a.Lk, Lq = a.Lq;
+    __bf16* sV = sm16 + wave * fwd16s_wave_elems<DKT>();
+    __bf16* sP = sV + KJS * PD;
+    float* sMask = reinterpret_cast<float*>(sP + 16 * PJS);
+    const int lr = lane & 15, lq = lane >> 4;
+    int64_t qrow0 = (int64_t)g * Lq;
+    int Lqg = Lq;
+    if (a.q_off) {
+        const int o0 = a.q_off[(int64_t)g * a.q_off_stride], o1 = a.q_off[(int64_t)(g + 1) * a.q_off_stride];
+        qrow0 = o0; Lqg = min(Lq, o1 - o0);
+    }
+    const int64_t krow0 = (a.q_off && a.kv_ragged) ? qrow0 : (int64_t)g * Lk;
+    const int Lkg = (a.q_off && a.kv_ragged) ? min(Lk, Lqg) : Lk;
+    bf16x8 vreg[DKT / 16];
+    stage32_ld<DKT>(vreg, av + krow0 * a.ldv + h * DK, a.ldv, Lkg, lane);
+    const float mk = (lane < Lkg) ? (a.kmask ? a.kmask[krow0 + lane] : 1.f) : -1.f;
+    RegRowFrags<NJT, NKS> kf;
+    ld_row_frags<NJT, NKS>(kf, ak + krow0 * a.ldk + h * DK, a.ldk, Lkg, lane);
+    bf16x8 qf[2][NKS];
+    float4 bias4[2][NJT];
+    int64_t prow[2], drow[2];
+    bool iv[2];
+#pragma unroll
+    for (int it = 0; it < 2; ++it) {
+        const int i = it * 16 + lr;
+        iv[it] = i < Lqg;
+        prow[it] = (((int64_t)g * a.H + h) * Lq + i) * Lk;
+        drow[it] = prow[it];
+        if (a.drop_p > 0.f && a.drop_rows && a.q_off && iv[it])
+            drow[it] = (((int64_t)g * a.H + h) * Lq + ((int64_t)a.drop_rows[qrow0 + i] - (int64_t)g * Lq)) * Lk;
+#pragma unroll
+        for (int ks = 0; ks < NKS; ++ks) qf[it][ks] = (bf16x8){0, 0, 0, 0, 0, 0, 0, 0};
+        if (iv[it]) {
+            const __bf16* qp = aq + (qrow0 + i) * a.ldq + h * DK + 8 * lq;
+#pragma unroll
+            for (int ks = 0; ks < NKS; ++ks) qf[it][ks] = ld_frag(qp + 32 * ks);
+        }
+        ld_keys4<NJT>(bias4[it], a.bias, a.bias && iv[it], prow[it], Lk, lq);
+    }
+    stage32_st<DKT>(sV, vreg, lane);
+    if (lane < 32) sMask[lane] = mk;
+    for (int idx = lane; idx < 16 * (KJS / 4); idx += 64)
+        *reinterpret_cast<bf16x4*>(sP + (idx / (KJS / 4)) * PJS + (idx % (KJS / 4)) * 4) = cvt4(make_float4(0.f, 0.f, 0.f, 0.f));
+    wsync();
+    const float inv_keep = a.drop_p > 0.f ? 1.f / (1.f - a.drop_p) : 1.f;
+#pragma unroll
+    for (int it = 0; it < 2; ++it) {
+        if (it * 16 >= Lqg) break;
+        fwd16_tile<NJT, DKT, PJS>(a, kf, qf[it], bias4[it], sMask, sV, sP, lane, it * 16 + lr, iv[it], prow[it], drow[it],
+                                  qrow0 + it * 16 + lr, h, inv_keep);
         wsync();
-        bf16x8 pf[KJ / 32];
-#pragma unroll
-        for (int ks = 0; ks < KJ / 32; ++ks) pf[ks] = frag_row<PJ>(sP, lr, 32 * ks + 8 * lq);
-#pragma unroll
-        for (int dt = 0; dt < DK / 16; ++dt) {
-            f32x4 o = (f32x4){0.f, 0.f, 0.f, 0.f};
-#pragma unroll
-            for (int ks = 0; ks < KJ / 32; ++ks) o = mma(frag_tr<PD>(sV, 32 * ks, 16 * dt, lane), pf[ks], o);
-            if (iv) st_elem4(a.o, (qrow0 + i) * a.ldo + h * DK + 16 * dt + 4 * lq, a.o_dtype, make_float4(o[0], o[1], o[2], o[3]));
-        }
     }
 }
 static int key_kj(int njt) { return njt <= 2 ? 32 : njt <= 4 ? 64 : njt <= 6 ? 96 : 128; }
@@ -177,10 +295,83 @@
     return ((size_t)(16 * njt + key_kj(njt)) * (dk + 8) + (size_t)16 * nw * key_pj(njt)) * sizeof(__bf16) + 128 * sizeof(float);
 }
 
+template <int NJT, int DKT, int PJ, typename VF>
+__device__ __forceinline__ void bwd16_tile1(const ortk_attn_args& a, const VF& vfr, const bf16x8 (&gf)[DKT / 32], const float4 (&praw)[NJT],
+                                            const __bf16* sK, __bf16* sS, __bf16* sD, int lane, int i, bool iv,
+                                            int64_t prow, int64_t drow, int64_t qrow, int h, float inv_keep) {
+    constexpr int DK = DKT, PD = DKT + 8, KJ = KeyGeo<NJT>::KJ;
+    const float qscale = DKT == 64 ? 0.125f : 0.17677669529663687f;
+    const int lq = lane >> 4, Lk = a.Lk;
+    const bool vec_p = (Lk & 3) == 0;
+    f32x4 dp[NJT], pp[NJT];
+    float dot = 0.f;
+#pragma unroll
+    for (int jt = 0; jt < NJT; ++jt) {
+        dp[jt] = (f32x4){0.f, 0.f, 0.f, 0.f};
+#pragma unroll
+        for (int ks = 0; ks < DK / 32; ++ks) dp[jt] = mma(vfr(jt, ks), gf[ks], dp[jt]);
+        const int j0 = 16 * jt + 4 * lq;
+        const float pv[4] = {praw[jt].x, praw[jt].y, praw[jt].z, praw[jt].w};
+        float pd[4];
+        bool kp[4] = {true, true, true, true};
+        if (a.drop_p > 0.f) ortk_keep4(a.drop_seed, (uint64_t)(drow + j0), a.drop_p, kp);
+#pragma unroll
+        for (int r = 0; r < 4; ++r) {
+            const bool valid = iv && j0 + r < Lk;
+            const bool keep = valid && kp[r];
+            const float d = keep ? dp[jt][r] * inv_keep : 0.f;
+            pd[r] = keep ? pv[r] * inv_keep : 0.f;
+            pp[jt][r] = valid ? pv[r] : 0.f; dp[jt][r] = d; dot += pp[jt][r] * d;
+        }
+        *reinterpret_cast<bf16x4*>(sD + i * PJ + j0) = cvt4(make_float4(pd[0], pd[1], pd[2], pd[3]));
+    }
+    dot += __shfl_xor(dot, 16, 64); dot += __shfl_xor(dot, 32, 64);
+#pragma unroll
+    for (int jt = 0; jt < NJT; ++jt) {
+        const int j0 = 16 * jt + 4 * lq;
+        float ds[4];
+#pragma unroll
+        for (int r = 0; r < 4; ++r) ds[r] = pp[jt][r] * (dp[jt][r] - dot);
+        if (a.dscore && iv) {
+            if (vec_p && j0 < Lk) *reinterpret_cast<float4*>(a.dscore + prow + j0) = make_float4(ds[0], ds[1], ds[2], ds[3]);
+            else for (int r = 0; r < 4; ++r) if (j0 + r < Lk) a.dscore[prow + j0 + r] = ds[r];
+        }
+        *reinterpret_cast<bf16x4*>(sS + i * PJ + j0) = cvt4(make_float4(ds[0] * qscale, ds[1] * qscale, ds[2] * qscale, ds[3] * qscale));
+    }
+    wsync();
+    bf16x8 sf[KJ / 32];
+#pragma unroll
+    for (int ks = 0; ks < KJ / 32; ++ks) sf[ks] = frag_row<PJ>(sS, i, 32 * ks + 8 * lq);
+#pragma unroll
+    for (int dt = 0; dt < DK / 16; ++dt) {
+        f32x4 acc = (f32x4){0.f, 0.f, 0.f, 0.f};
+#pragma unroll
+        for (int ks = 0; ks < KJ / 32; ++ks) acc = mma(frag_tr<PD>(sK, 32 * ks, 16 * dt, lane), sf[ks], acc);
+        if (iv) st_elem4(a.dq, qrow * a.lddq + h * DK + 16 * dt + 4 * lq, a.dqkv_dtype, make_float4(acc[0], acc[1], acc[2], acc[3]));
+    }
+}
+template <int NJT, int DKT, int PJ>
+__device__ __forceinline__ void bwd16_tile2(const ortk_attn_args& a, int t, const __bf16* sS, const __bf16* sD, const __bf16* sQ, const __bf16* sG,
+                                            int Lqp, int lane, int Lkg, int64_t krow0, int h) {
+    constexpr int DK = DKT, PD = DKT + 8, NDT = DK / 16;
+    const int lr = lane & 15, lq = lane >> 4;
+    const int which = t / (NJT * NDT), rem = t - which * NJT * NDT, jt = rem / NDT, dt = rem % NDT;
+    const __bf16* sA = which == 0 ? sS : sD;
+    const __bf16* sB = which == 0 ? sQ : sG;
+    f32x4 acc = (f32x4){0.f, 0.f, 0.f, 0.f};
+    for (int k0 = 0; k0 < Lqp; k0 += 32) acc = mma(frag_tr<PD>(sB, k0, 16 * dt, lane), frag_tr<PJ>(sA, k0, 16 * jt, lane), acc);
+    const int j = 16 * jt + lr;
+    if (j < Lkg) {
+        const int64_t row = krow0 + j;
+        const float4 v = make_float4(acc[0], acc[1], acc[2], acc[3]);
+        if (which == 0) st_elem4(a.d_k, row * a.lddk + h * DK + 16 * dt + 4 * lq, a.dqkv_dtype, v);
+        else            st_elem4(a.dv, row * a.lddv + h * DK + 16 * dt + 4 * lq, a.dqkv_dtype, v);
+    }
+}
+
 template <int NJT, typename TQ, int DKT>
 __global__ __launch_bounds__(512) void attn16_bwd_kernel(ortk_attn_args a, int Lqp) {
     constexpr int DK = DKT, PD = DKT + 8;
-    const float qscale = DKT == 64 ? 0.125f : 0.17677669529663687f;
     const TQ* aq = reinterpret_cast<const TQ*>(a.q); const TQ* ak = reinterpret_cast<const TQ*>(a.k); const TQ* av = reinterpret_cast<const TQ*>(a.v);
     extern __shared__ __attribute__((aligned(16))) __bf16 sm16[];
     const int tid = threadIdx.x, lane = tid & 63, wave = tid >> 6, nw = blockDim.x >> 6;
@@ -194,7 +385,6 @@
     __bf16* sS = sG + Lqp * PD;
     __bf16* sD = sS + Lqp * PJ;
     const int lr = lane & 15, lq = lane >> 4;
-    const bool vec_p = (Lk & 3) == 0;
     const int nit = (Lq + 15) >> 4;
     const int64_t qrow0 = a.q_off ? (int64_t)a.q_off[(int64_t)g * a.q_off_stride] : (int64_t)g * Lq;
     const int Lqg = a.q_off ? min(Lq, (int)(a.q_off[(int64_t)(g + 1) * a.q_off_stride] - qrow0)) : Lq;
@@ -207,15 +397,7 @@
     const int64_t drow = (a.drop_rows && a.q_off && iv && a.drop_p > 0.f)
                              ? (((int64_t)g * a.H + h) * Lq + ((int64_t)a.drop_rows[qrow0 + i] - (int64_t)g * Lq)) * Lk : prow;
     float4 praw[NJT];
-#pragma unroll
-    for (int jt = 0; jt < NJT; ++jt) {
-        const int j0 = 16 * jt + 4 * lq;
-        praw[jt] = make_float4(0.f, 0.f, 0.f, 0.f);
-        if (iv) {
-            if (vec_p && j0 < Lk) praw[jt] = *reinterpret_cast<const float4*>(a.p + prow + j0);
-            else { float* q = &praw[jt].x; for (int r = 0; r < 4; ++r) if (j0 + r < Lk) q[r] = a.p[prow + j0 + r]; }
-        }
-    }
+    ld_keys4<NJT>(praw, a.p, iv, prow, Lk, lq);
     stage_rows<DK>(sK, ak + krow0 * a.ldk + h * DK, a.ldk, Lkg, KJ, tid, blockDim.x);
     stage_rows<DK>(sV, av + krow0 * a.ldv + h * DK, a.ldv, Lkg, 16 * NJT, tid, blockDim.x);
     stage_rows<DK>(sQ, aq + qrow0 * a.ldq + h * DK, a.ldq, Lqg, Lqp, tid, blockDim.x);
@@ -228,69 +410,84 @@
         bf16x8 gf[DK / 32];
 #pragma unroll
         for (int ks = 0; ks < DK / 32; ++ks) gf[ks] = frag_row<PD>(sG, i, 32 * ks + 8 * lq);
-        f32x4 dp[NJT], pp[NJT];
-        float dot = 0.f;
-#pragma unroll
-        for (int jt = 0; jt < NJT; ++jt) {
-            dp[jt] = (f32x4){0.f, 0.f, 0.f, 0.f};
-#pragma unroll
-            for (int ks = 0; ks < DK / 32; ++ks) dp[jt] = mma(frag_row<PD>(sV, 16 * jt + lr, 32 * ks + 8 * lq), gf[ks], dp[jt]);
-            const int j0 = 16 * jt + 4 * lq;
-            const float pv[4] = {praw[jt].x, praw[jt].y, praw[jt].z, praw[jt].w};
-            float pd[4];
-            bool kp[4] = {true, true, true, true};
-            if (a.drop_p > 0.f) ortk_keep4(a.drop_seed, (uint64_t)(drow + j0), a.drop_p, kp);
-#pragma unroll
-            for (int r = 0; r < 4; ++r) {
-                const bool valid = iv && j0 + r < Lk;
-                const bool keep = valid && kp[r];
-                const float d = keep ? dp[jt][r] * inv_keep : 0.f;
-                pd[r] = keep ? pv[r] * inv_keep : 0.f;
-                pp[jt][r] = valid ? pv[r] : 0.f; dp[jt][r] = d; dot += pp[jt][r] * d;
-            }
-            *reinterpret_cast<bf16x4*>(sD + i * PJ + j0) = cvt4(make_float4(pd[0], pd[1], pd[2], pd[3]));
-        }
-        dot += __shfl_xor(dot, 16, 64); dot += __shfl_xor(dot, 32, 64);
-#pragma unroll
-        for (int jt = 0; jt < NJT; ++jt) {
-            const int j0 = 16 * jt + 4 * lq;
-            float ds[4];
-#pragma unroll
-            for (int r = 0; r < 4; ++r) ds[r] = pp[jt][r] * (dp[jt][r] - dot);
-            if (a.dscore && iv) {
-                if (vec_p && j0 < Lk) *reinterpret_cast<float4*>(a.dscore + prow + j0) = make_float4(ds[0], ds[1], ds[2], ds[3]);
-                else for (int r = 0; r < 4; ++r) if (j0 + r < Lk) a.dscore[prow + j0 + r] = ds[r];
-            }
-            *reinterpret_cast<bf16x4*>(sS + i * PJ + j0) = cvt4(make_float4(ds[0] * qscale, ds[1] * qscale, ds[2] * qscale, ds[3] * qscale));
-        }
+        bwd16_tile1<NJT, DKT, PJ>(a, LdsRowFrags<PD>{sV, lr, lq}, gf, praw, sK, sS, sD, lane, i, iv, prow, drow, qrow0 + i, h, inv_keep);
+    }
+    __syncthreads();
+    for (int t = wave; t < 2 * NJT * (DK / 16); t += nw) bwd16_tile2<NJT, DKT, PJ>(a, t, sS, sD, sQ, sG, Lqp, lane, Lkg, krow0, h);
+}
+
+template <int DKT> constexpr int bwd16s_wave_elems() { return 32 * (DKT + 8) + 2 * 32 * PJS; }
+template <int NJT, int DKT>
+__global__ __launch_bounds__(512) void attn16s_bwd_kernel(ortk_attn_args a) {
+    static_assert(NJT <= 2, "the short kernels serve at most 32 keys");
+    constexpr int DK = DKT, PD = DKT + 8, NKS = DKT / 32, LQP = 32;
+    const __bf16* aq = reinterpret_cast<const __bf16*>(a.q); const __bf16* ak = reinterpret_cast<const __bf16*>(a.k); const __bf16* av = reinterpret_cast<const __bf16*>(a.v);
+    const __bf16* ag = reinterpret_cast<const __bf16*>(a.d_o);
+    extern __shared__ __attribute__((aligned(16))) __bf16 sm16[];
+    const int lane = threadIdx.x & 63, wave = __builtin_amdgcn_readfirstlane((int)(threadIdx.x >> 6)), W = blockDim.x >> 6;
+    const int pair = blockIdx.x * W + wave;
+    if (pair >= a.nkv * a.H) return;
+    const int g = pair / a.H, h = pair - g * a.H;
+    const int Lk = a.Lk, Lq = a.Lq;
+    __bf16* sX = sm16 + wave * bwd16s_wave_elems<DKT>();
+    __bf16* sS = sX + 32 * PD;
+    __bf16* sD = sS + LQP * PJS;
+    const int lr = lane & 15, lq = lane >> 4;
+    int64_t qrow0 = (int64_t)g * Lq;
+    int Lqg = Lq;
+    if (a.q_off) {
+        const int o0 = a.q_off[(int64_t)g * a.q_off_stride], o1 = a.q_off[(int64_t)(g + 1) * a.q_off_stride];
+        qrow0 = o0; Lqg = min(Lq, o1 - o0);
+    }
+    const int64_t krow0 = (a.q_off && a.kv_ragged) ? qrow0 : (int64_t)g * Lk;
+    const int Lkg = (a.q_off && a.kv_ragged) ? min(Lk, Lqg) : Lk;
+    RegRowFrags<NJT, NKS> vf;
+    ld_row_frags<NJT, NKS>(vf, av + krow0 * a.ldv + h * DK, a.ldv, Lkg, lane);
+    bf16x8 gf[2][NKS];
+    float4 praw[2][NJT];
+    int64_t prow[2], drow[2];
+    bool iv[2];
+#pragma unroll
+    for (int it = 0; it < 2; ++it) {
+        const int i = it * 16 + lr;
+        iv[it] = i < Lqg;
+        prow[it] = (((int64_t)g * a.H + h) * Lq + i) * Lk;
+        drow[it] = prow[it];
+        if (a.drop_p > 0.f && a.drop_rows && a.q_off && iv[it])
+            drow[it] = (((int64_t)g * a.H + h) * Lq + ((int64_t)a.drop_rows[qrow0 + i] - (int64_t)g * Lq)) * Lk;
+#pragma unroll
+        for (int ks = 0; ks < NKS; ++ks) gf[it][ks] = (bf16x8){0, 0, 0, 0, 0, 0, 0, 0};
+        if (iv[it]) {
+            const __bf16* gp = ag + (qrow0 + i) * a.lddo + h * DK + 8 * lq;
+#pragma unroll
+            for (int ks = 0; ks < NKS; ++ks) gf[it][ks] = ld_frag(gp + 32 * ks);
+        }
+        ld_keys4<NJT>(praw[it], a.p, iv[it], prow[it], Lk, lq);
+    }
+    bf16x8 kreg[DKT / 16], qreg[DKT / 16], greg[DKT / 16];
+    stage32_ld<DKT>(kreg, ak + krow0 * a.ldk + h * DK, a.ldk, Lkg, lane);
+    stage32_ld<DKT>(qreg, aq + qrow0 * a.ldq + h * DK, a.ldq, Lqg, lane);
+    stage32_ld<DKT>(greg, ag + qrow0 * a.lddo + h * DK, a.lddo, Lqg, lane);
+    for (int idx = lane; idx < 2 * LQP * PJS / 8; idx += 64)
+        *reinterpret_cast<bf16x8*>(sS + idx * 8) = (bf16x8){0, 0, 0, 0, 0, 0, 0, 0};
+    stage32_st<DKT>(sX, kreg, lane);
+    wsync();
+    const float inv_keep = a.drop_p > 0.f ? 1.f / (1.f - a.drop_p) : 1.f;
+#pragma unroll
+    for (int it = 0; it < 2; ++it) {
+        if (it * 16 >= Lqg) break;
+        bwd16_tile1<NJT, DKT, PJS>(a, vf, gf[it], praw[it], sX, sS, sD, lane, it * 16 + lr, iv[it], prow[it], drow[it],
+                                   qrow0 + it * 16 + lr, h, inv_keep);
+    }
+    constexpr int NDT = DK / 16;
+#pragma unroll
+    for (int which = 0; which < 2; ++which) {
         wsync();
-        bf16x8 sf[KJ / 32];
-#pragma unroll
-        for (int ks = 0; ks < KJ / 32; ++ks) sf[ks] = frag_row<PJ>(sS, i, 32 * ks + 8 * lq);
-#pragma unroll
-        for (int dt = 0; dt < DK / 16; ++dt) {
-            f32x4 acc = (f32x4){0.f, 0.f, 0.f, 0.f};
-#pragma unroll
-            for (int ks = 0; ks < KJ / 32; ++ks) acc = mma(frag_tr<PD>(sK, 32 * ks, 16 * dt, lane), sf[ks], acc);
-            if (iv) st_elem4(a.dq, (qrow0 + i) * a.lddq + h * DK + 16 * dt + 4 * lq, a.dqkv_dtype, make_float4(acc[0], acc[1], acc[2], acc[3]));
-        }
-    }
-    __syncthreads();
-    constexpr int NDT = DK / 16;
-    const int ntiles = 2 * NJT * NDT;
-    for (int t = wave; t < ntiles; t += nw) {
-        const int which = t / (NJT * NDT), rem = t - which * NJT * NDT, jt = rem / NDT, dt = rem % NDT;
-        const __bf16* sA = which == 0 ? sS : sD;
-        const __bf16* sB = which == 0 ? sQ : sG;
-        f32x4 acc = (f32x4){0.f, 0.f, 0.f, 0.f};
-        for (int k0 = 0; k0 < Lqp; k0 += 32) acc = mma(frag_tr<PD>(sB, k0, 16 * dt, lane), frag_tr<PJ>(sA, k0, 16 * jt, lane), acc);
-        const int j = 16 * jt + lr;
-        if (j < Lkg) {
-            const int64_t row = krow0 + j;
-            const float4 v = make_float4(acc[0], acc[1], acc[2], acc[3]);
-            if (which == 0) st_elem4(a.d_k, row * a.lddk + h * DK + 16 * dt + 4 * lq, a.dqkv_dtype, v);
-            else            st_elem4(a.dv, row * a.lddv + h * DK + 16 * dt + 4 * lq, a.dqkv_dtype, v);
-        }
+        stage32_st<DKT>(sX, which == 0 ? qreg : greg, lane);
+        wsync();
+        for (int jt = 0; jt < NJT && 16 * jt < Lkg; ++jt)
+            for (int dt = 0; dt < NDT; ++dt)
+                bwd16_tile2<NJT, DKT, PJS>(a, (which * NJT + jt) * NDT + dt, sS, sD, sX, sX, LQP, lane, Lkg, krow0, h);
     }
 }
 static size_t bwd16_lds(int njt, int Lqp, int dk) {
@@ -340,7 +537,26 @@
     }
 }
 
+static int short_waves(const ortk_attn_args* a) {
+    const int sw = ortk::tuning().attn16_short;
+    if (!sw || a->qkv_dtype != 1 || a->Lq > 32 || a->Lk > 32) return 0;
+    return sw == 8 ? 8 : 4;
+}
+template <typename FN> static int launch_short(FN fn, size_t wave_bytes, int W, const ortk_attn_args* a, hipStream_t s) {
+    const size_t lds = wave_bytes * W;
+    const int64_t pairs = (int64_t)a->nkv * a->H;
+    if (lds > 64 * 1024) ortk::lds_attr(reinterpret_cast<const void*>(fn), 160 * 1024);
+    hipLaunchKernelGGL(fn, dim3((unsigned)((pairs + W - 1) / W)), dim3(64 * W), lds, s, *a);
+    ORTK_CHECK_LAUNCH();
+    return 0;
+}
+
 int attn16_fwd(const ortk_attn_args* a, hipStream_t s) {
+    if (const int W = short_waves(a)) {
+        const bool two = a->Lk > 16;
+        const fwd16_fn fn = a->dk == 64 ? (two ? attn16s_fwd_kernel<2, 64> : attn16s_fwd_kernel<1, 64>) : (two ? attn16s_fwd_kernel<2, 32> : attn16s_fwd_kernel<1, 32>);
+        return launch_short(fn, (a->dk == 64 ? fwd16s_wave_elems<64>() : fwd16s_wave_elems<32>()) * sizeof(__bf16), W, a, s);
+    }
     const int njt = (a->Lk + 15) / 16, nw = (a->Lq + 15) / 16;
     const fwd16_fn fn = a->dk == 64 ? (a->qkv_dtype ? pick_fwd<__bf16, 64>(njt) : pick_fwd<float, 64>(njt))
                                     : (a->qkv_dtype ? pick_fwd<__bf16, 32>(njt) : pick_fwd<float, 32>(njt));
@@ -352,6 +568,11 @@
 }
 
 int attn16_bwd(const ortk_attn_args* a, hipStream_t s) {
+    if (const int W = short_waves(a)) {
+        const bool two = a->Lk > 16;
+        const fwd16_fn fn = a->dk == 64 ? (two ? attn16s_bwd_kernel<2, 64> : attn16s_bwd_kernel<1, 64>) : (two ? attn16s_bwd_kernel<2, 32> : attn16s_bwd_kernel<1, 32>);
+        return launch_short(fn, (a->dk == 64 ? bwd16s_wave_elems<64>() : bwd16s_wave_elems<32>()) * sizeof(__bf16), W, a, s);
+    }
     const int njt = (a->Lk + 15) / 16, nw = (a->Lq + 15) / 16, Lqp = (int)ortk_align(a->Lq, 32);
     const bwd16_fn fn = a->dk == 64 ? (a->qkv_dtype ? pick_bwd<__bf16, 64>(njt) : pick_bwd<float, 64>(njt))
                                     : (a->qkv_dtype ? pick_bwd<__bf16, 32>(njt) : pick_bwd<float, 32>(njt));
diff --git a/sparse-image-captioning_amd/csrc/ortk_runtime.hip b/sparse-image-captioning_amd/csrc/ortk_runtime.hip
--- a/sparse-image-captioning_amd/csrc/ortk_runtime.hip
+++ b/sparse-image-captioning_amd/csrc/ortk_runtime.hip
@@ -22,6 +22,7 @@
     t.ln_fuse = 0;
     t.samp_epilogue = 1;
     t.gemm_epilogue = 0;
+    t.attn16_short = 1;
     return t;
 }
 static ortk_tuning g_tuning = tuning_defaults();
@@ -35,7 +36,8 @@
     if (!in(t->attn_impl, 0, 4) || t->attn16_min_lq < 1 || !in(t->f32_split, 0, 7) || t->wgrad_wgs < 1 ||
         !in(t->wgrad_group, 0, 15) || !in(t->wgrad_group_splitk, 0, 8) || t->wgrad_group_wgs < 1 || !in(t->wgrad_group_tail, 0, 1) ||
         !in(t->feats_bf16, 0, 1) || !in(t->ln_fuse, 0, 15) || (t->ln_fuse & 2)  ||
-        !in(t->samp_epilogue, 0, 1) || !in(t->gemm_epilogue, 0, 3)) return ORTK_EINVAL;
+        !in(t->samp_epilogue, 0, 1) || !in(t->gemm_epilogue, 0, 3) ||
+        !(in(t->attn16_short, 0, 1) || t->attn16_short == 4 || t->attn16_short == 8)) return ORTK_EINVAL;
     ortk::g_tuning = *t;
     return 0;
 }
```

After: 130,900 captions/sec (median of 6 runs). +2.3%, better.
